# aantoine890/navierstokes

Measured on AMD Instinct MI355X. Metric: fp64 CSR SpMV GFLOP/s & % HBM roofline @ nnz; 1/2/4/8 GPU, higher is better.
Workload: dtype f64

## Files before the change

### include/mi355_devtools.h

```cpp
#ifndef MI355_DEVTOOLS_H
#define MI355_DEVTOOLS_H
#include "mi355_spmv.h"
#ifdef __cplusplus
extern "C" {
#endif
int mi_debug_xcc_map(int wgs, int* host_out);
int mi_debug_touch_pages(mi_csr_t A, int stride_bytes, const void* d_extra0, long long bytes0, const void* d_extra1, long long bytes1);
int mi_debug_mring_trace(mi_csr_t A, const double* d_x, double* d_y, int max_wgs, long long* host_out, int* wgs_out);
int mi_debug_move_array(mi_csr_t A, int which, int how, unsigned long long* old_ptr, unsigned long long* new_ptr);
int mi_debug_mring_replan(mi_csr_t A, int skew_pct, int* table_len, int* longest_run);
int mi_debug_part_push_trace(mi_part_t P, double* d_x_ext, double* d_y_local, int max_wgs, long long* host_out, int* wgs_out, int* halo_out);
int mi_debug_part_ext_mode(mi_part_t P, int mode);
int mi_debug_part_ext_trace(mi_part_t P, double* d_x_ext, double* d_y_local, int max_wgs, long long* host_out, int* wgs_out, int* modes_out);
int mi_part_push_debug_preset(mi_part_t P, unsigned value);

#ifdef __cplusplus
}
#endif
#endif
```

### navierstokes_amd/csrc/capi_bcsr.hip

```cpp
#include "capi_internal.hpp"
#include "spmv_bcsr_sell.hpp"

static int sell_fill(mi_bcsr4_t A, hipStream_t s);

template <class Select>
static bool bcsr4_race(mi_bcsr4_t A, int ncand, Select select, double* us)
{
    LaunchTimer tm;
    ScratchPair sp;
    if (sp.alloc(4 * (size_t)std::max(A->nbcols, 1), 4 * (size_t)std::max(A->nbrows, 1)) != MI_OK || tm.init() != MI_OK) return false;
    std::vector<char> failed((size_t)ncand, 0);
    for (int round = 0; round < 2; round++)
        for (int c = 0; c < ncand; c++) {
            if (failed[c]) continue;
            select(c);
            double t = 0.0;
            if (tm.time(3, 8, [&] { return launch_bcsr4(A, sp.x, sp.y, nullptr, false); }, &t) == MI_OK) us[c] = min_measured(us[c], t);
            else failed[c] = 1;
        }
    for (int c = 0; c < ncand; c++)
        if (failed[c]) us[c] = 0.0;
    return true;
}

// ... 68 lines not shown
    A->sell_nsteps = P.nsteps;
    return sell_fill(A, nullptr);
}

static void choose_bcsr4_sell_form(mi_bcsr4_t A, bool forced)
{
    if (const char* fe = getenv("MI355_BCSR_SELL_FORM")) A->sell_form = std::max(0, std::min(3, atoi(fe)));
    else if (forced) A->sell_form = 0;
    else if (env_is("MI355_SPMV_AUTOTUNE", "0")) A->sell_form = 0;
    else {
        double us[5] = {0, 0, 0, 0, 0};
        if (!bcsr4_race(A, 5, [&](int c) { A->sell_form = c - 1; }, us)) return;
        int best = 0;
        for (int c = 1; c < 5; c++) {
            A->tune_us_sell[c - 1] = us[c];
            if (better(us[c], us[best])) best = c;
        }
        if (A->tune_us_plain <= 0 && A->tune_us_tile <= 0) A->tune_us_plain = us[0];
        A->sell_form = best - 1;
    }
}

extern "C" int mi_bcsr4_create(int nbrows, int nbcols, const int* ptrow, const int* indcol, const double* coef,
                               mi_bcsr4_t* out)
{
    CHECK_ARG(out, "out is null");
    *out = nullptr;
    CHECK_ARG(nbrows >= 0 && nbcols >= 0 && ptrow && ptrow[0] == 0, "bad argument");
    for (int i = 0; i < nbrows; i++) CHECK_ARG(ptrow[i] <= ptrow[i + 1], "ptrow must be non-decreasing");
    const long long nb = ptrow[nbrows];
    CHECK_ARG(nb == 0 || (indcol && coef), "indcol/coef is null");
    for (long long k = 0; k < nb; k++) CHECK_ARG(indcol[k] >= 0 && indcol[k] < nbcols, "block column outside [0, nbcols)");
    int rc = need_device();
    if (rc) return rc;
    std::unique_ptr<mi_bcsr4_s, int (*)(mi_bcsr4_t)> owner(new (std::nothrow) mi_bcsr4_s(), mi_bcsr4_destroy);
    mi_bcsr4_t A = owner.get();
    if (!A) return fail(MI_ERR_ALLOC, "host allocation failed");
    A->nbrows = nbrows;
    A->nbcols = nbcols;
    A->nblocks = nb;
    hipError_t e;
    if ((e = hipGetDevice(&A->device)) != hipSuccess ||
        (e = hipMalloc(&A->d_ptrow, sizeof(int) * ((size_t)nbrows + 1))) != hipSuccess ||
        (e = hipMalloc(&A->d_indcol, sizeof(int) * ((size_t)nb + 1))) != hipSuccess ||
        (e = hipMalloc(&A->d_coef, sizeof(double) * 16 * ((size_t)nb + 1))) != hipSuccess ||
        (e = hipMemcpy(A->d_ptrow, ptrow, sizeof(int) * ((size_t)nbrows + 1), hipMemcpyHostToDevice)) != hipSuccess ||
        (nb && (e = hipMemcpy(A->d_indcol, indcol, sizeof(int) * (size_t)nb, hipMemcpyHostToDevice)) != hipSuccess) ||
        (nb && (e = hipMemcpy(A->d_coef, coef, sizeof(double) * 16 * (size_t)nb, hipMemcpyHostToDevice)) != hipSuccess))
        return fail(e == hipErrorOutOfMemory ? MI_ERR_ALLOC : MI_ERR_HIP, std::string("bcsr4 upload: ") + hipGetErrorString(e));
    for (int s0 = 0; s0 < nbrows; s0 += kSellRows)
        A->max_slice_vals = std::max(A->max_slice_vals, 16 * (ptrow[std::min(nbrows, s0 + kSellRows)] - ptrow[s0]));
    if ((rc = build_bcsr4_tile(A, ptrow, indcol))) return rc;
    const bool forced = env_is("MI355_BCSR_SELL", "1");
    if (!env_is("MI355_BCSR_SELL", "0") && (forced || nb >= 100000) && nbcols > 0 && nbcols < (1 << 30)) {
        if ((rc = build_bcsr4_sell(A, ptrow, indcol))) return rc;
        if (A->d_sell_val) choose_bcsr4_sell_form(A, forced);
    }
    if ((e = hipStreamSynchronize(nullptr)) != hipSuccess) return fail(MI_ERR_HIP, std::string("mi_bcsr4_create: ") + hipGetErrorString(e));
    *out = owner.release();
    return MI_OK;
}

static int sell_fill(mi_bcsr4_t A, hipStream_t s)
{
    const int grid = std::max(1, std::min(A->sell_nslices, 8192));
    hipLaunchKernelGGL(bcsr4_to_sell_kernel, dim3((unsigned)grid), dim3(64), 0, s, A->sell_nslices, A->nbrows, A->d_ptrow, A->d_coef, A->d_sell_sptr, A->d_sell_val);
    HIP_TRY(hipGetLastError());
    return MI_OK;
}

int bcsr4_refresh_from_csr(mi_bcsr4_s* A, const int* d_csr_ptrow, const double* d_src, double* d_csr_out, hipStream_t s)
{
    if (!A || A->nbrows == 0) return MI_OK;
    const int nslices = (A->nbrows + kSellRows - 1) / kSellRows;
    const int grid = std::max(1, std::min(nslices, 2048));
    const int* sptr = A->d_sell_val ? A->d_sell_sptr : nullptr;
    double* sv = A->d_sell_val;
    if (A->max_slice_vals <= 4096)
        hipLaunchKernelGGL((bcsr4_refresh_kernel<4096>), dim3((unsigned)grid), dim3(256), 0, s, nslices, A->nbrows, d_csr_ptrow, d_src, d_csr_out, A->d_ptrow, A->d_coef, sptr, sv);
    else if (A->max_slice_vals <= 16384)
        hipLaunchKernelGGL((bcsr4_refresh_kernel<16384>), dim3((unsigned)std::min(grid, 256)), dim3(256), 0, s, nslices, A->nbrows, d_csr_ptrow, d_src, d_csr_out, A->d_ptrow, A->d_coef, sptr, sv);
    else
        hipLaunchKernelGGL((bcsr4_refresh_kernel<0>), dim3((unsigned)grid), dim3(256), 0, s, nslices, A->nbrows, d_csr_ptrow, d_src, d_csr_out, A->d_ptrow, A->d_coef, sptr, sv);
    HIP_TRY(hipGetLastError());
    return MI_OK;
}

static int bcsr4_refresh_from_blocks(mi_bcsr4_s* A, const double* d_src, bool colmajor, hipStream_t s)
{
    if (!A || A->nbrows == 0 || A->nblocks == 0) return MI_OK;
    const int nslices = (A->nbrows + kSellRows - 1) / kSellRows;
    const int grid = std::max(1, std::min(nslices, 2048));
    const int* sptr = A->d_sell_val ? A->d_sell_sptr : nullptr;
    double* out = d_src == A->d_coef ? nullptr : A->d_coef;
    if (colmajor && !out) return fail(MI_ERR_ARG, "column-major blocks cannot be transposed in place");
    if (!out && !A->d_sell_val) return MI_OK;
#define BR_LAUNCH(CAP_, CM_, G_) hipLaunchKernelGGL((bcsr4_blocks_refresh_kernel<CAP_, CM_>), dim3((unsigned)(G_)), dim3(256), 0, s, nslices, A->nbrows, A->d_ptrow, d_src, out, sptr, A->d_sell_val)
    if (A->max_slice_vals <= 4096) { if (colmajor) BR_LAUNCH(4096, true, grid); else BR_LAUNCH(4096, false, grid); }
    else if (A->max_slice_vals <= 16384) { if (colmajor) BR_LAUNCH(16384, true, std::min(grid, 256)); else BR_LAUNCH(16384, false, std::min(grid, 256)); }
    else { if (colmajor) BR_LAUNCH(0, true, grid); else BR_LAUNCH(0, false, grid); }
#undef BR_LAUNCH
    HIP_TRY(hipGetLastError());
    return MI_OK;
}

int bcsr4_values_changed(mi_bcsr4_s* A, hipStream_t s)
{
    if (A && A->d_sell_val && A->nblocks > 0) return sell_fill(A, s);
    return MI_OK;
}

extern "C" int mi_bcsr4_sell_info(mi_bcsr4_t A, int* built, int* form_in_use, long long* steps, double* padding, double us[4])
{
    CHECK_ARG(A, "null handle");
    if (built) *built = A->d_sell_val != nullptr;
    if (form_in_use) *form_in_use = A->d_sell_val ? A->sell_form : -1;
    if (steps) *steps = A->sell_nsteps;
    if (padding) *padding = A->nblocks > 0 && A->d_sell_val ? (double)A->sell_nsteps * kSellRows / (double)A->nblocks - 1.0 : 0.0;
    if (us)
        for (int i = 0; i < 4; i++) us[i] = A->tune_us_sell[i];
    return MI_OK;
}

extern "C" int mi_bcsr4_sell_plan_probe(int nbrows, const int* ptrow, const int* indcol, int nwaves_max, int* nslices, long long* nsteps,
                                        int* nwaves, int* sptr, int* wrng, unsigned* col)
{
    CHECK_ARG(nbrows >= 0 && ptrow && ptrow[0] == 0 && nwaves_max >= 1, "bad argument");
    for (int i = 0; i < nbrows; i++) CHECK_ARG(ptrow[i] <= ptrow[i + 1], "ptrow must be non-decreasing");
    const long long nb = ptrow[nbrows];
    CHECK_ARG(nb == 0 || indcol, "indcol is null");
    for (long long k = 0; k < nb; k++) CHECK_ARG(indcol[k] >= 0 && indcol[k] < (1 << 30), "block column outside [0, 2^30)");
    SellPlanHost P;
    build_sell_plan(nbrows, ptrow, indcol, nwaves_max, P);
    if (nslices) *nslices = P.nslices;
    if (nsteps) *nsteps = P.nsteps;
    if (nwaves) *nwaves = P.nwaves;
    if (sptr) std::copy(P.sptr.begin(), P.sptr.end(), sptr);
    if (wrng) std::copy(P.wrng.begin(), P.wrng.end(), wrng);
    if (col) std::copy(P.col.begin(), P.col.end(), col);
    return MI_OK;
}

static void transpose_blocks_host(long long nb, const double* src, double* dst)
{
    for (long long k = 0; k < nb; k++)
        for (int r = 0; r < 4; r++)
            for (int c = 0; c < 4; c++) dst[16 * k + 4 * r + c] = src[16 * k + 4 * c + r];
}

extern "C" int mi_bcsr4_create_layout(int nbrows, int nbcols, const int* ptrow, const int* indcol, const double* coef, int layout,
                                      mi_bcsr4_t* out)
{
    CHECK_ARG(layout == MI_BLOCK_ROWMAJOR || layout == MI_BLOCK_COLMAJOR, "unknown block layout");
    if (layout == MI_BLOCK_ROWMAJOR) return mi_bcsr4_create(nbrows, nbcols, ptrow, indcol, coef, out);
    CHECK_ARG(out, "out is null");
    *out = nullptr;
    CHECK_ARG(nbrows >= 0 && ptrow && ptrow[0] == 0 && ptrow[nbrows] >= 0, "bad argument");
    const long long nb = ptrow[nbrows];
    CHECK_ARG(nb == 0 || coef, "coef is null");
    std::vector<double> t((size_t)nb * 16);
    transpose_blocks_host(nb, coef, t.data());
    return mi_bcsr4_create(nbrows, nbcols, ptrow, indcol, t.data(), out);
}

extern "C" int mi_bcsr4_update_values_layout(mi_bcsr4_t A, const double* coef, int layout)
{
// ... 605 lines not shown
```

### navierstokes_amd/csrc/capi_csr.hip

```cpp
#include "capi_internal.hpp"
#include "reorder.hpp"
#include "mring_plan.hpp"
#include "tile_plan.hpp"

int get_table(mi_csr_t A, int nnzb, BlockTable** out)
{
    BlockTable& T = A->tables[nnzb];
    if (!T.d_blk) {
        std::vector<int> rows, ptrs;
        int row_align = A->nnz < 20000000 ? 64 : 1;
        if (const char* e = getenv("MI355_STREAM_ROW_ALIGN")) row_align = std::max(1, atoi(e));
        build_row_blocks(A->n, A->h_ptrow.data(), nnzb, 4 * kWG, rows, ptrs, row_align, 7);
        T.nnzb = nnzb;
        T.nblk = (int)rows.size() - 1;
        std::vector<int2> h(rows.size());
        for (size_t i = 0; i < rows.size(); i++) h[i] = make_int2(rows[i], ptrs[i]);
        HIP_TRY(hipMalloc(&T.d_blk, sizeof(int2) * h.size()));
        HIP_TRY(hipMemcpy(T.d_blk, h.data(), sizeof(int2) * h.size(), hipMemcpyHostToDevice));
    }
    *out = &T;
    return MI_OK;
}

static void free_tile(mi_csr_t A)
{
    dfree(A->tile.d_desc);
    dfree(A->tile.d_ulist);
    dfree(A->tile.d_slots);
    A->tile = TileTable();
}

static void free_mring(mi_csr_t A)
{
    dfree(A->mring.d_plan);
    dfree(A->mring.d_first);
    dfree(A->mring.d_ok);
    dfree(A->mring.d_rng);
    dfree(A->mring.d_slots);
    A->mring = MringTable();
}

static void free_sstream(mi_csr_t A)
{
    ss_free(A->ss.dev);
    A->ss = SstreamTable();
}

static inline bool beyond_infinity_cache(double bytes_per_nnz, long long nnz, int n) { return bytes_per_nnz * (double)nnz + 16.0 * (double)n > 0.75 * 256e6; }

constexpr double kSsMaxPadding = 0.12;
static double ss_max_padding()
{
    if (const char* e = getenv("MI355_SSTREAM_MAX_PADDING")) return std::max(0.0, atof(e));
    return kSsMaxPadding;
}

static int build_sstream(mi_csr_t A, const int* ptrow, const int* indcol, int ghost_lo = 0, int ghost_hi = 0)
{
    if (A->ss.dev.val) return MI_OK;
    SsPlanHost P;
    SsMwPlanHost M;
    const int shift = (A->y_offset & 1) && !A->d_rowmap ? 1 : 0;
    build_sstream_plan(A->n, A->ncols, ptrow, indcol, ss_max_padding(), P, true, shift, ghost_lo, ghost_hi);
    SstreamTable& T = A->ss;
    hipError_t e;
    if (!P.eligible) {
        if (ghost_lo < ghost_hi || env_is("MI355_SSTREAM_MW", "0")) return MI_OK;
        build_sstream_mw_plan(A->n, A->ncols, ptrow, indcol, ss_max_padding(), M, shift);
        if (!M.eligible) return MI_OK;
        e = ss_mw_upload(M, T.dev);
        T.mw = e == hipSuccess;
    } else e = ss_upload(P, T.dev, ghost_lo < ghost_hi);
    const SsPlanHost& Q = P.eligible ? P : M;
    if (e != hipSuccess) {
        free_sstream(A);
        if (e == hipErrorOutOfMemory) { (void)hipGetLastError(); return MI_OK; }
        return fail(MI_ERR_HIP, std::string("sliced copy: ") + hipGetErrorString(e));
    }
    T.nwg = Q.nwg;
    T.rounds = Q.rounds;
    T.shift = Q.shift;
    T.steps = Q.steps;
    T.padding = (double)Q.pad_places / (double)A->nnz;
    T.max_slice_nnz = Q.max_slice_nnz;
    if (ghost_lo < ghost_hi) {
        T.h_wg_halo = P.wg_halo;
        T.h_wg = P.wg;
        T.fusable = P.fusable;
    }
    sstream_fill_values(T.rounds, A->n, T.shift, A->d_ptrow, A->d_coef, nullptr, T.dev.slice_step, T.dev.slice_len, T.dev.val, T.max_slice_nnz, nullptr, T.mw ? 1 : 0);
    if ((e = hipGetLastError()) != hipSuccess) {
        free_sstream(A);
        return fail(MI_ERR_HIP, std::string("sliced copy fill: ") + hipGetErrorString(e));
    }
    T.nt = beyond_infinity_cache(10.0, A->nnz, A->n);
    T.deep = T.nt;
    if (const char* fe = getenv("MI355_SSTREAM_FORM")) {
        const int f = atoi(fe);
        T.nt = (f & 1) == 0;
        T.deep = f >= 2;
    }
    return MI_OK;
}

int launch_sstream(mi_csr_t A, const double* d_x, double* d_y, const int* rowmap, hipStream_t s, const RingComm* comm)
{
    SstreamTable& T = A->ss;
    SsView S{T.dev.val, T.dev.slot, T.dev.wg, T.dev.win, T.nwg, A->n + T.shift, A->ncols, rowmap, T.shift};
    double* yy = rowmap ? d_y : d_y - T.shift;
    if (T.mw) {
        if (comm) return fail(MI_ERR_STATE, "the cut-ring sliced stream has no fused multi-GPU form");
        SsMwView V{S, T.dev.winK};
        if (T.deep) {
            if (T.nt) hipLaunchKernelGGL((spmv_sstream_mw<12, true>), dim3((unsigned)T.nwg), dim3(256), 0, s, V, d_x, yy);
            else hipLaunchKernelGGL((spmv_sstream_mw<12, false>), dim3((unsigned)T.nwg), dim3(256), 0, s, V, d_x, yy);
        } else {
            if (T.nt) hipLaunchKernelGGL((spmv_sstream_mw<8, true>), dim3((unsigned)T.nwg), dim3(256), 0, s, V, d_x, yy);
            else hipLaunchKernelGGL((spmv_sstream_mw<8, false>), dim3((unsigned)T.nwg), dim3(256), 0, s, V, d_x, yy);
        }
        HIP_TRY(hipGetLastError());
        return MI_OK;
    }
    if (comm) {
        const unsigned grid = (unsigned)(T.nwg + comm->push_wgs);
        if (T.deep) {
            if (T.nt) hipLaunchKernelGGL((spmv_sstream_fused<12, true>), dim3(grid), dim3(256), 0, s, S, d_x, yy, *comm);
            else hipLaunchKernelGGL((spmv_sstream_fused<12, false>), dim3(grid), dim3(256), 0, s, S, d_x, yy, *comm);
        } else {
            if (T.nt) hipLaunchKernelGGL((spmv_sstream_fused<8, true>), dim3(grid), dim3(256), 0, s, S, d_x, yy, *comm);
            else hipLaunchKernelGGL((spmv_sstream_fused<8, false>), dim3(grid), dim3(256), 0, s, S, d_x, yy, *comm);
        }
    } else if (T.deep) {
        if (T.nt) hipLaunchKernelGGL((spmv_sstream<12, true>), dim3((unsigned)T.nwg), dim3(256), 0, s, S, d_x, yy);
        else hipLaunchKernelGGL((spmv_sstream<12, false>), dim3((unsigned)T.nwg), dim3(256), 0, s, S, d_x, yy);
    } else {
        if (T.nt) hipLaunchKernelGGL((spmv_sstream<8, true>), dim3((unsigned)T.nwg), dim3(256), 0, s, S, d_x, yy);
        else hipLaunchKernelGGL((spmv_sstream<8, false>), dim3((unsigned)T.nwg), dim3(256), 0, s, S, d_x, yy);
    }
    HIP_TRY(hipGetLastError());
    return MI_OK;
}

static bool ring_wants_skew(int n, const int* ptrow)
{
    long long bad = 0;
    for (int i = 0; i < n; i++) {
        const int len = ptrow[i + 1] - ptrow[i];
        bad += len > 0 && (len % 16 == 0 || len == 8);
    }
    return 2 * bad > n;
}

constexpr long long kLargeNnz = 20000000;
static size_t placed_vector_len(int n, int ncols) { return (size_t)std::max(n, ncols) + 64; }
static int large_row_align(long long nnz) { return nnz >= kLargeNnz ? 1 : 0; }

static int build_mring(mi_csr_t A, const int* indcol, int row_align = 0)
{
    if (A->mring.d_plan || A->n == 0 || A->nnz == 0) return MI_OK;
    std::vector<int> back;
    if (!indcol) {
        if (!A->d_indcol) return fail(MI_ERR_STATE, "mring plan: the handle no longer holds its column indices");
        back.resize((size_t)A->nnz);
        HIP_TRY(hipMemcpy(back.data(), A->d_indcol, sizeof(int) * (size_t)A->nnz, hipMemcpyDeviceToHost));
        indcol = back.data();
    }
    MringPlanHost P;
    build_mring_plan(A->n, A->h_ptrow.data(), indcol, P, row_align);
    MringTable& M = A->mring;
    hipError_t e;
    if ((e = hipMalloc(&M.d_plan, sizeof(int) * P.plan.size())) != hipSuccess ||
        (e = hipMalloc(&M.d_first, sizeof(int) * P.first.size())) != hipSuccess ||
        (e = hipMemcpy(M.d_first, P.first.data(), sizeof(int) * P.first.size(), hipMemcpyHostToDevice)) != hipSuccess ||
// ... 92 lines not shown
    RING_TRY(hipMemcpy(R.d_plan, best.plan.data(), sizeof(int) * best.plan.size(), hipMemcpyHostToDevice));
    RING_TRY(hipMalloc(&R.d_ok, sizeof(int) * best.run_ok.size()));
    RING_TRY(hipMemcpy(R.d_ok, best.run_ok.data(), sizeof(int) * best.run_ok.size(), hipMemcpyHostToDevice));
    R.all_in_loop = true;
    for (int g = 0; g < best.wgs; g++) R.all_in_loop = R.all_in_loop && best.run_ok[g] == 1;
    R.h_dep_ptr.clear();
    R.h_dep_run.clear();
    if (square && row_min && R.all_in_loop && R.lean && best.cfg.id == 4 && !ghosts) build_run_deps(best, n, R.h_dep_ptr, R.h_dep_run);
    for (int g = 0; g < best.wgs; g++)
        R.uniform = R.uniform && best.run_rng[2 * g] == std::min(best.nblk, g * best.bpw) &&
                    best.run_rng[2 * g + 1] == std::min(best.nblk, (g + 1) * best.bpw);
    RING_TRY(hipMalloc(&R.d_rng, sizeof(int) * best.run_rng.size()));
    RING_TRY(hipMemcpy(R.d_rng, best.run_rng.data(), sizeof(int) * best.run_rng.size(), hipMemcpyHostToDevice));
    if (ghosts) {
        R.h_run_halo = best.run_halo;
        RING_TRY(hipMalloc(&R.d_run_halo, sizeof(int) * best.run_halo.size()));
        RING_TRY(hipMemcpy(R.d_run_halo, best.run_halo.data(), sizeof(int) * best.run_halo.size(), hipMemcpyHostToDevice));
    }
    {
        std::vector<unsigned short> slots;
        build_ring_slots(best, indcol, slots);
        RING_TRY(hipMalloc(&R.d_slots, sizeof(unsigned short) * slots.size()));
        RING_TRY(hipMemcpy(R.d_slots, slots.data(), sizeof(unsigned short) * slots.size(), hipMemcpyHostToDevice));
    }
#undef RING_TRY
    R.skew = ring_wants_skew(n, ptrow);
    if (const char* e2 = getenv("MI355_RING_SKEW")) R.skew = atoi(e2) != 0;
    return MI_OK;
}

static int time_on(LaunchTimer& tm, mi_csr_t A, const double* x, double* y, int warm, int timed, double* us)
{
    return tm.time(warm, timed, [&] { return launch_spmv(A, x, y, nullptr); }, us);
}

static int placement_draws(mi_csr_t A, double* tx, double* ty, bool keep_pair)
{
    const long long nnz = A->nnz;
    const char* pe = getenv("MI355_PLACEMENT_DRAWS");
    int draws = pe ? std::max(0, std::min(16, atoi(pe))) : 4;
    const bool early_stop = pe == nullptr;
    if (!pe) {
        size_t mem_free = 0, mem_total = 0;
        if (hipMemGetInfo(&mem_free, &mem_total) == hipSuccess && nnz > 0)
            draws = (int)std::min<size_t>((size_t)draws, mem_free / 8 / (sizeof(double) * (size_t)nnz));
        else (void)hipGetLastError();
    }
    const bool blocked_choice = A->auto_kernel == MI_KERNEL_BCSR4 && A->blocked && A->blocked->d_coef && !(A->blocked->sell_form >= 0 && A->blocked->d_sell_val);
    const bool streams_coef = A->auto_kernel == MI_KERNEL_RING || A->auto_kernel == MI_KERNEL_MRING || A->auto_kernel == MI_KERNEL_STREAM || A->auto_kernel == MI_KERNEL_TILE || blocked_choice;
    if (!(draws > 0 && streams_coef && nnz >= kLargeNnz)) return MI_OK;
    LaunchTimer tm;
    ScratchPair own;
    if (!tx || !ty) {
        const size_t len = std::max(placed_vector_len(A->n, A->ncols), (size_t)(A->n_out > 0 ? A->n_out : 1));
        if (int rc = own.alloc(len, len)) return rc;
        tx = own.x;
        ty = own.y;
    }
    if (int rc = tm.init()) return rc;
    auto time_now = [&](double* us) { return time_on(tm, A, tx, ty, 3, 8, us); };
    auto redraw = [&](void** slot, size_t bytes, size_t pad_bytes, int ndraws) {
        double best = 0.0;
        if (!*slot || bytes == 0 || time_now(&best) != MI_OK) return;
        const double first = best;
        A->place_us.push_back(best);
        std::vector<void*> losers;
        for (int d = 0; d < ndraws; d++) {
            void* fresh = nullptr;
            if (hipMalloc(&fresh, bytes + pad_bytes) != hipSuccess) { (void)hipGetLastError(); break; }
            if ((pad_bytes && hipMemset((char*)fresh + bytes, 0, pad_bytes) != hipSuccess) ||
                hipMemcpy(fresh, *slot, bytes, hipMemcpyDeviceToDevice) != hipSuccess) { (void)hipGetLastError(); dfree(fresh); break; }
            std::swap(*slot, fresh);
            double t = 0.0;
            const int rct = time_now(&t);
            A->place_us.push_back(rct == MI_OK ? t : -1.0);
            if (rct == MI_OK && t < 0.96 * best) best = t;
            else std::swap(*slot, fresh);
            losers.push_back(fresh);
            if (early_stop && d == 0 && rct == MI_OK && std::fabs(t - first) <= 0.02 * first) break;
        }
        for (void* l : losers) dfree(l);
    };
    if (blocked_choice) redraw((void**)&A->blocked->d_coef, sizeof(double) * 16 * (size_t)A->blocked->nblocks, sizeof(double) * 16, draws);
    else redraw((void**)&A->d_coef, sizeof(double) * (size_t)nnz, sizeof(double) * (size_t)kRingPadNnz, draws);
    A->place_draws_coef = (int)A->place_us.size();
    if (A->auto_kernel == MI_KERNEL_RING) redraw((void**)&A->ring.d_slots, sizeof(unsigned short) * (size_t)A->ring.nblk * A->ring.cfg.nnzb, 0, (draws + 1) / 2);
    else if (A->auto_kernel == MI_KERNEL_MRING) redraw((void**)&A->mring.d_slots, sizeof(unsigned short) * (size_t)A->mring.nblk * kMringNnzb, 0, (draws + 1) / 2);
    if (keep_pair && !A->kept_x) {
        A->kept_x = tx;
        A->kept_y = ty;
        if (tx == own.x) own.hand_over();
    }
    return MI_OK;
}

constexpr long long kMeasureNnz = 200000;

struct CsrInput {
    int n, ncols;
    const int* ptrow;
    const int* indcol;
    const double* coef;
    const int* rowmap;
    int ghost_lo, ghost_hi;
    long long nnz = 0;
    bool offset_only = false;
    std::vector<int> row_min, row_max;
    bool ghosts() const { return ghost_lo < ghost_hi; }
};

static int check_input(CsrInput& in)
{
    const int n = in.n;
    const int* ptrow = in.ptrow;
    CHECK_ARG(n >= 0 && in.ncols >= 0, "negative dimension");
    CHECK_ARG(ptrow, "ptrow is null");
    CHECK_ARG(ptrow[0] == 0, "ptrow[0] must be 0");
    for (int i = 0; i < n; i++) CHECK_ARG(ptrow[i] <= ptrow[i + 1], "ptrow must be non-decreasing");
    in.nnz = ptrow[n];
    CHECK_ARG(in.nnz == 0 || (in.indcol && in.coef), "indcol/coef is null");
    CHECK_ARG(in.nnz <= 0x7fffffffLL - 2 * kRingPadNnz && n <= 0x7fffffff - 2 * kRingPadRows, "matrix too large for 32-bit offsets: partition it (mi_part_*)");
    in.row_min.resize((size_t)n);
    in.row_max.resize((size_t)n);
    for (int i = 0; i < n; i++) {
        int lo = 0x7fffffff, hi = -1;
        for (int k = ptrow[i]; k < ptrow[i + 1]; k++) {
            const int c = in.indcol[k];
            CHECK_ARG(c >= 0 && c < in.ncols, "column index outside [0, ncols)");
            lo = c < lo ? c : lo;
            hi = c > hi ? c : hi;
        }
        in.row_min[i] = lo;
        in.row_max[i] = hi;
    }
    in.offset_only = in.rowmap != nullptr && n > 0;
    for (int i = 1; in.offset_only && i < n; i++) in.offset_only = in.rowmap[i] == in.rowmap[0] + i;
    return MI_OK;
}

static int upload(mi_csr_t A, const CsrInput& in)
{
    const int n = in.n;
    const long long nnz = in.nnz;
    const size_t pad = 8, padv = kRingPadNnz, padr = kRingPadRows;
    HIP_TRY(hipGetDevice(&A->device));
    HIP_TRY(hipMalloc(&A->d_ptrow, sizeof(int) * ((size_t)n + 1 + padr)));
    HIP_TRY(hipMalloc(&A->d_indcol, sizeof(int) * ((size_t)nnz + pad)));
    HIP_TRY(hipMalloc(&A->d_coef, sizeof(double) * ((size_t)nnz + padv)));
    HIP_TRY(hipMemset(A->d_ptrow + n + 1, 0, sizeof(int) * padr));
    HIP_TRY(hipMemset(A->d_indcol + nnz, 0, sizeof(int) * pad));
    HIP_TRY(hipMemset(A->d_coef + nnz, 0, sizeof(double) * padv));
    HIP_TRY(hipMemcpy(A->d_ptrow, in.ptrow, sizeof(int) * ((size_t)n + 1), hipMemcpyHostToDevice));
    if (nnz) {
        HIP_TRY(hipMemcpy(A->d_indcol, in.indcol, sizeof(int) * (size_t)nnz, hipMemcpyHostToDevice));
        HIP_TRY(hipMemcpy(A->d_coef, in.coef, sizeof(double) * (size_t)nnz, hipMemcpyHostToDevice));
    }
    A->mapped = in.rowmap != nullptr;
    if (in.offset_only) A->y_offset = in.rowmap[0];
    if (in.rowmap && n > 0 && !in.offset_only) {
        HIP_TRY(hipMalloc(&A->d_rowmap, sizeof(int) * ((size_t)n + padr)));
        HIP_TRY(hipMemset(A->d_rowmap + n, 0, sizeof(int) * padr));
        HIP_TRY(hipMemcpy(A->d_rowmap, in.rowmap, sizeof(int) * (size_t)n, hipMemcpyHostToDevice));
    }
    return MI_OK;
}

static int plan_ring(mi_csr_t A, const CsrInput& in)
// ... 203 lines not shown
static void compare_ring_shapes(mi_csr_t A, const CsrInput& in, LaunchTimer& tm, const ScratchPair& sp)
{
    const long long nnz = in.nnz;
    if (!env_is("MI355_RING_SHAPE_COMPARE", "1") || getenv("MI355_RING_ROW_ALIGN") || nnz < kLargeNnz) return;
    auto time_now = [&](double* us) { return time_on(tm, A, sp.x, sp.y, 3, 8, us); };
    double us64 = 0.0, us1 = 0.0;
    if (A->auto_kernel == MI_KERNEL_RING && A->ring.cfg.id == 4) {
        RingPlanHost alt;
        build_ring_plan(kRingConfigs[3], in.n, in.ptrow, in.row_min.data(), in.row_max.data(), alt, in.ghost_lo, in.ghost_hi, 64);
        RingTable T2;
        if (1.0 - (double)alt.bad_nnz / (double)nnz >= 0.90 &&
            fill_ring_table(T2, alt, in.n, in.ptrow, in.indcol, nnz, in.ghosts(), in.row_min.data(), in.row_max.data(), in.n == in.ncols) == MI_OK) {
            T2.nt = A->ring.nt;
            A->kernel = MI_KERNEL_RING;
            int rct = time_now(&us1);
            std::swap(A->ring, T2);
            if (rct == MI_OK) rct = time_now(&us64);
            A->kernel = MI_KERNEL_AUTO;
            A->tune_us_ring_aligned = us64;
            A->tune_us_ring_unaligned = us1;
            if (rct != MI_OK || !(us64 < 0.98 * us1)) std::swap(A->ring, T2);
            free_ring_table(T2);
        }
    } else if (A->auto_kernel == MI_KERNEL_MRING) {
        MringTable keep = A->mring;
        A->mring = MringTable();
        if (build_mring(A, in.indcol, 64) == MI_OK && A->mring.d_plan && A->mring.ok_fraction >= 0.90) {
            A->mring.nt = keep.nt;
            A->kernel = MI_KERNEL_MRING;
            int rct = time_now(&us64);
            std::swap(A->mring, keep);
            if (rct == MI_OK) rct = time_now(&us1);
            A->kernel = MI_KERNEL_AUTO;
            A->tune_us_ring_aligned = us64;
            A->tune_us_ring_unaligned = us1;
            if (rct == MI_OK && us64 < 0.98 * us1) std::swap(A->mring, keep);
        } else {
            std::swap(A->mring, keep);
        }
        std::swap(A->mring, keep);
        free_mring(A);
        A->mring = keep;
    }
}

static int measure_at_create(mi_csr_t A, const CsrInput& in, bool defer_placement)
{
    const size_t scratch_len = placed_vector_len(in.n, in.ncols);
    LaunchTimer tm;
    ScratchPair sp;
    int rc = sp.alloc(std::max(scratch_len, (size_t)(in.ncols > 0 ? in.ncols : 1)), std::max(scratch_len, (size_t)(A->n_out > 0 ? A->n_out : 1)));
    if (rc || (rc = tm.init())) return rc;
    tune(A, tm, sp);
    compare_ring_shapes(A, in, tm, sp);
    if (!defer_placement && placement_draws(A, sp.x, sp.y, !in.rowmap && in.n == in.ncols && in.n == A->n_out && !in.ghosts()) == MI_OK &&
        A->kept_x == sp.x)
        sp.hand_over();
    return MI_OK;
}

int csr_create_impl(int n, int ncols, const int* ptrow, const int* indcol, const double* coef,
                    const int* rowmap, mi_csr_t* out, int ghost_lo, int ghost_hi, bool defer_placement)
{
    CHECK_ARG(out, "out is null");
    *out = nullptr;
    CsrInput in{n, ncols, ptrow, indcol, coef, rowmap, ghost_lo, ghost_hi};
    int rc = check_input(in);
    if (rc || (rc = need_device())) return rc;
    std::unique_ptr<mi_csr_s, int (*)(mi_csr_t)> owner(new (std::nothrow) mi_csr_s(), mi_csr_destroy);
    mi_csr_t A = owner.get();
    if (!A) return fail(MI_ERR_ALLOC, "host allocation failed");
    A->n = n;
    A->ncols = ncols;
    A->nnz = in.nnz;
    A->ghost_lo = ghost_lo;
    A->ghost_hi = ghost_hi;
    A->h_ptrow.assign(ptrow, ptrow + n + 1);
    if ((rc = upload(A, in)) || (rc = plan_ring(A, in)) || (rc = plan_optional(A, in)) || (rc = attach_blocked(A, in))) return rc;
    load_defaults(A, in);
    const bool forced_kernel = apply_forced_kernel(A);
    if (!forced_kernel && in.nnz < kMeasureNnz && A->auto_kernel == MI_KERNEL_RING && !in.ghosts()) A->auto_kernel = MI_KERNEL_STREAM;
    if (!forced_kernel && !env_is("MI355_SPMV_AUTOTUNE", "0") && in.nnz >= kMeasureNnz && (rc = measure_at_create(A, in, defer_placement))) return rc;
    HIP_TRY(hipStreamSynchronize(nullptr));
    *out = owner.release();
    return MI_OK;
}

static int time_handle(mi_csr_t A, int warm, int timed, double* us)
{
    LaunchTimer tm;
    ScratchPair sp;
    int rc = sp.alloc((size_t)(A->ncols > 0 ? A->ncols : 1), (size_t)(A->n_out > 0 ? A->n_out : 1));
    if (rc || (rc = tm.init())) return rc;
    return time_on(tm, A, sp.x, sp.y, warm, timed, us);
}

static void release_natural_arrays(mi_csr_t A)
{
    dfree(A->d_ptrow);
    dfree(A->d_indcol);
    dfree(A->d_coef);
    A->d_ptrow = A->d_indcol = nullptr;
    A->d_coef = nullptr;
    for (auto& kv : A->tables) dfree(kv.second.d_blk);
    A->tables.clear();
    free_ring_table(A->ring);
    free_tile(A);
    free_mring(A);
    free_sstream(A);
    mi_bcsr4_destroy(A->blocked);
    A->blocked = nullptr;
}

static int maybe_reorder(mi_csr_t A, const int* ptrow, const int* indcol, const double* coef)
{
    const bool force = env_is("MI355_REORDER", "1");
    if (env_is("MI355_REORDER", "0")) return MI_OK;
    const int n = A->n;
    if (A->mapped || n != A->ncols || n < 8 || A->nnz == 0) return MI_OK;
    if (!force && (n < 100000 || resolve_kernel(A) == MI_KERNEL_RING || resolve_kernel(A) == MI_KERNEL_SSTREAM)) return MI_OK;
    const int block = csr_has_block4_pattern(n, ptrow, indcol) ? 4 : 1;
    const double nn = (double)n / block;
    const double spread = mean_column_distance(n, ptrow, indcol, block);
    A->spread_before = spread;
    if (!force && spread < 2.0 * std::pow(nn, 2.0 / 3.0)) return MI_OK;
    Reorder R;
    rcm_reorder(n, ptrow, indcol, block, R);
    A->reorder_block = block;
    A->spread_after = R.spread_after;
    if (!force && R.spread_after > 0.5 * spread) return MI_OK;
    std::vector<int> p2, c2, src_start;
    std::vector<double> v2;
    permute_csr(n, ptrow, indcol, coef, R, p2, c2, v2, src_start);
    mi_csr_t inner = nullptr;
    int rc = csr_create_impl(n, n, p2.data(), c2.data(), v2.data(), R.iperm.data(), &inner);
    if (rc) return rc;
    A->inner = inner;
    hipError_t e;
    if ((e = hipMalloc(&A->d_iperm, sizeof(int) * (size_t)n)) != hipSuccess ||
        (e = hipMalloc(&A->d_src_start, sizeof(int) * (size_t)n)) != hipSuccess ||
        (e = hipMalloc(&A->d_xp, sizeof(double) * (size_t)n)) != hipSuccess ||
        (e = hipMemcpy(A->d_iperm, R.iperm.data(), sizeof(int) * (size_t)n, hipMemcpyHostToDevice)) != hipSuccess ||
        (e = hipMemcpy(A->d_src_start, src_start.data(), sizeof(int) * (size_t)n, hipMemcpyHostToDevice)) != hipSuccess)
        return fail(e == hipErrorOutOfMemory ? MI_ERR_ALLOC : MI_ERR_HIP, std::string("reorder upload: ") + hipGetErrorString(e));
    bool keep = true;
    if (!force && !env_is("MI355_SPMV_AUTOTUNE", "0")) {
        const int timed = A->nnz < 40000000 ? 12 : 6;
        A->inner = nullptr;
        rc = time_handle(A, 3, timed, &A->us_natural);
        A->inner = inner;
        if (rc) return rc;
        if ((rc = time_handle(A, 3, timed, &A->us_reordered))) return rc;
        keep = A->us_reordered < 0.97 * A->us_natural;
    }
    if (!keep) {
        mi_csr_destroy(A->inner);
        A->inner = nullptr;
        dfree(A->d_iperm);
        dfree(A->d_src_start);
        dfree(A->d_xp);
        A->d_iperm = A->d_src_start = nullptr;
        A->d_xp = nullptr;
        return MI_OK;
    }
    A->h_iperm = R.iperm;
    A->xp_claimed = false;
    release_natural_arrays(A);
    return MI_OK;
}

extern "C" int mi_csr_create(int n, int ncols, const int* ptrow, const int* indcol, const double* coef, mi_csr_t* out)
{
    int rc = csr_create_impl(n, ncols, ptrow, indcol, coef, nullptr, out, 0, 0, true);
    if (rc) return rc;
    if ((rc = maybe_reorder(*out, ptrow, indcol, coef)) || (!(*out)->inner && (rc = placement_draws(*out, nullptr, nullptr, n == ncols))) ||
        (hipStreamSynchronize(nullptr) != hipSuccess && (rc = fail(MI_ERR_HIP, "mi_csr_create: synchronize")))) {
        mi_csr_destroy(*out);
        *out = nullptr;
    }
    return rc;
}

extern "C" int mi_reorder_probe(int n, const int* ptrow, const int* indcol, int* block, int* perm, double* spread_before,
                                double* spread_after)
{
    CHECK_ARG(n >= 0 && ptrow && (ptrow[n] == 0 || indcol), "bad argument");
    for (int i = 0; i < n; i++) {
        CHECK_ARG(ptrow[i] <= ptrow[i + 1], "ptrow must be non-decreasing");
        for (int k = ptrow[i]; k < ptrow[i + 1]; k++) CHECK_ARG(indcol[k] >= 0 && indcol[k] < n, "column index outside [0, n)");
    }
    const int b = csr_has_block4_pattern(n, ptrow, indcol) ? 4 : 1;
    Reorder R;
    rcm_reorder(n, ptrow, indcol, b, R);
    if (block) *block = b;
    if (perm)
        for (int i = 0; i < n; i++) perm[i] = R.perm[i];
    if (spread_before) *spread_before = R.spread_before;
    if (spread_after) *spread_after = R.spread_after;
    return MI_OK;
}

extern "C" int mi_csr_reorder_info(mi_csr_t A, int* reordered, int* block, double* spread_before, double* spread_after,
                                   double* us_natural, double* us_reordered)
{
    CHECK_ARG(A, "null handle");
    if (reordered) *reordered = A->inner ? 1 : 0;
    if (block) *block = A->reorder_block;
    if (spread_before) *spread_before = A->spread_before;
    if (spread_after) *spread_after = A->spread_after;
    if (us_natural) *us_natural = A->us_natural;
    if (us_reordered) *us_reordered = A->us_reordered;
    return MI_OK;
}

extern "C" int mi_csr_perm(mi_csr_t A, int* reordered, int* perm)
{
    CHECK_ARG(A, "null handle");
    if (reordered) *reordered = A->inner ? 1 : 0;
    if (perm) {
        if (A->inner) {
            CHECK_ARG((int)A->h_iperm.size() == A->n, "permutation not kept on this handle");
            for (int r = 0; r < A->n; r++) perm[A->h_iperm[r]] = r;
        } else {
            for (int i = 0; i < A->n; i++) perm[i] = i;
        }
    }
    return MI_OK;
}

extern "C" int mi_vec_to_internal_dev(mi_csr_t A, const double* d_x, double* d_x_int, mi_stream_t s)
{
    CHECK_ARG(A, "null handle");
    if (A->n == 0) return MI_OK;
    CHECK_ARG(d_x && d_x_int && d_x != d_x_int, "null vector, or in place");
    if (A->inner) return gather_perm(A, d_x, d_x_int, (hipStream_t)s);
    HIP_TRY(hipMemcpyAsync(d_x_int, d_x, sizeof(double) * (size_t)A->n, hipMemcpyDeviceToDevice, (hipStream_t)s));
    return MI_OK;
}

extern "C" int mi_vec_from_internal_dev(mi_csr_t A, const double* d_x_int, double* d_x, mi_stream_t s)
{
    CHECK_ARG(A, "null handle");
    if (A->n == 0) return MI_OK;
    CHECK_ARG(d_x && d_x_int && d_x != d_x_int, "null vector, or in place");
    if (A->inner) return scatter_perm(A, d_x_int, d_x, (hipStream_t)s);
    HIP_TRY(hipMemcpyAsync(d_x, d_x_int, sizeof(double) * (size_t)A->n, hipMemcpyDeviceToDevice, (hipStream_t)s));
    return MI_OK;
}

extern "C" int mi_spmv_internal_dev(mi_csr_t A, const double* d_x_int, double* d_y_int, mi_stream_t s)
{
    CHECK_ARG(A, "null handle");
    CHECK_ARG(A->n == A->ncols && !A->mapped, "the internal numbering is defined for square, unmapped matrices");
    CHECK_ARG(A->n == 0 || (d_x_int && d_y_int), "null vector");
    if (A->inner) return launch_spmv(A->inner, d_x_int, d_y_int, (hipStream_t)s, false);
    return launch_spmv(A, d_x_int, d_y_int, (hipStream_t)s);
}

extern "C" int mi_spmk_internal_dev(mi_csr_t A, int k, const double* d_x_int, double* const* d_y_int_out, mi_stream_t s)
{
    CHECK_ARG(A, "null handle");
    if (k < 1 || k > MI_MAX_POWERS) return fail(MI_ERR_UNSUPPORTED, "k must be in 1..MI_MAX_POWERS");
    CHECK_ARG(d_y_int_out, "null output array");
    CHECK_ARG(A->n == A->ncols && !A->mapped, "the internal numbering is defined for square, unmapped matrices");
    if (A->n == 0) return MI_OK;
    CHECK_ARG(d_x_int, "null vector");
    for (int p = 0; p < k; p++) CHECK_ARG(d_y_int_out[p], "null output vector");
    return spmk_unmapped(A->inner ? A->inner : A, k, d_x_int, d_y_int_out, (hipStream_t)s);
}

extern "C" int mi_csr_create_mapped(int n, int ncols, const int* ptrow, const int* indcol, const double* coef,
                                    const int* rowmap, mi_csr_t* out)
{
    return csr_create_impl(n, ncols, ptrow, indcol, coef, rowmap, out);
}

extern "C" int mi_csr_destroy(mi_csr_t A)
{
    if (!A) return MI_OK;
    dfree(A->d_ptrow);
    dfree(A->d_indcol);
    dfree(A->d_coef);
    dfree(A->d_rowmap);
    dfree(A->d_x);
    dfree(A->d_y);
    dfree(A->kept_x);
    dfree(A->kept_y);
    for (double* p : A->d_pow) dfree(p);
    for (auto& kv : A->tables) {
        dfree(kv.second.d_blk);
    }
    free_ring_table(A->ring);
    free_tile(A);
    free_mring(A);
    free_sstream(A);
    mi_bcsr4_destroy(A->blocked);
    mi_csr_destroy(A->inner);
    dfree(A->d_iperm);
    dfree(A->d_src_start);
    dfree(A->d_xp);
    for (auto& kv : A->xp_more) dfree(kv.second);
    dfree(A->d_vtmp);
    for (double* p : A->d_pp) dfree(p);
    spmk_release(A);
    delete A;
    return MI_OK;
}

static int refresh_blocked_values(mi_csr_t A, hipStream_t s, bool sliced_done = false)
{
    if (A->ss.dev.val && !sliced_done) {
        SstreamTable& T = A->ss;
        sstream_fill_values(T.rounds, A->n, T.shift, A->d_ptrow, A->d_coef, nullptr, T.dev.slice_step, T.dev.slice_len, T.dev.val, T.max_slice_nnz, s, T.mw ? 1 : 0);
        HIP_TRY(hipGetLastError());
    }
    if (!A->blocked || A->blocked->nbrows == 0) return MI_OK;
    return bcsr4_refresh_from_csr(A->blocked, A->d_ptrow, A->d_coef, nullptr, s);
}

__global__ __launch_bounds__(256) void permute_values_kernel(int n, const int* __restrict__ new_ptrow, const int* __restrict__ src_start,
                                                             const double* __restrict__ src, double* __restrict__ dst)
{
    __shared__ int s_p[65], s_a[64];
    const int tid = threadIdx.x;
    for (int r0 = blockIdx.x * 64; r0 < n; r0 += gridDim.x * 64) {
        const int nr = min(64, n - r0);
        if (tid <= nr) s_p[tid] = new_ptrow[r0 + tid];
        if (tid < nr) s_a[tid] = src_start[r0 + tid];
        __syncthreads();
        const int b0 = s_p[0], seg = s_p[nr] - b0;
        for (int k = tid; k < seg; k += 256) {
            const int p = b0 + k;
            int lo = 0, hi = nr;
            while (hi - lo > 1) {
                const int mid = (lo + hi) >> 1;
                if (s_p[mid] <= p) lo = mid;
                else hi = mid;
            }
            dst[p] = src[s_a[lo] + (p - s_p[lo])];
        }
        __syncthreads();
    }
}

extern "C" int mi_csr_update_values_dev(mi_csr_t A, const double* d_coef, mi_stream_t s_)
{
    CHECK_ARG(A, "null handle");
    if (A->nnz == 0) return MI_OK;
    CHECK_ARG(d_coef, "null coef");
    hipStream_t s = (hipStream_t)s_;
    if (A->inner) {
        mi_csr_t I = A->inner;
        hipLaunchKernelGGL(permute_values_kernel, dim3((unsigned)std::max(1, std::min((A->n + 63) / 64, 4096))), dim3(256), 0, s, A->n, I->d_ptrow, A->d_src_start, d_coef, I->d_coef);
        HIP_TRY(hipGetLastError());
        return refresh_blocked_values(I, s);
    }
    if (A->ss.dev.val && d_coef != A->d_coef) {
        SstreamTable& T = A->ss;
        sstream_fill_values(T.rounds, A->n, T.shift, A->d_ptrow, d_coef, A->d_coef, T.dev.slice_step, T.dev.slice_len, T.dev.val, T.max_slice_nnz, s, T.mw ? 1 : 0);
        HIP_TRY(hipGetLastError());
        return refresh_blocked_values(A, s, true);
    }
    if (A->blocked && A->blocked->nbrows > 0 && d_coef != A->d_coef)
        return bcsr4_refresh_from_csr(A->blocked, A->d_ptrow, d_coef, A->d_coef, s);
    if (d_coef != A->d_coef) HIP_TRY(hipMemcpyAsync(A->d_coef, d_coef, sizeof(double) * (size_t)A->nnz, hipMemcpyDeviceToDevice, s));
    return refresh_blocked_values(A, s);
}

extern "C" int mi_csr_update_values(mi_csr_t A, const double* coef)
{
    CHECK_ARG(A, "null handle");
    if (A->nnz == 0) return MI_OK;
    CHECK_ARG(coef, "null coef");
    if (A->inner) {
        if (!A->d_vtmp) HIP_TRY(hipMalloc(&A->d_vtmp, sizeof(double) * (size_t)A->nnz));
        HIP_TRY(hipMemcpy(A->d_vtmp, coef, sizeof(double) * (size_t)A->nnz, hipMemcpyHostToDevice));
        int rc = mi_csr_update_values_dev(A, A->d_vtmp, nullptr);
        if (rc) return rc;
        HIP_TRY(hipStreamSynchronize(nullptr));
        return MI_OK;
    }
    HIP_TRY(hipMemcpy(A->d_coef, coef, sizeof(double) * (size_t)A->nnz, hipMemcpyHostToDevice));
    int rc = refresh_blocked_values(A, nullptr);
    if (rc) return rc;
    HIP_TRY(hipStreamSynchronize(nullptr));
    return MI_OK;
}

extern "C" int mi_csr_dims(mi_csr_t A, int* n, int* ncols, long long* nnz)
{
    CHECK_ARG(A, "null handle");
    if (n) *n = A->n;
    if (ncols) *ncols = A->ncols;
    if (nnz) *nnz = A->nnz;
    return MI_OK;
}

int resolve_kernel(const mi_csr_s* A)
{
    int k = A->kernel != MI_KERNEL_AUTO ? A->kernel : A->auto_kernel;
    if (k == MI_KERNEL_RING && !A->ring.d_plan) k = MI_KERNEL_STREAM;
    if (k == MI_KERNEL_BCSR4 && !A->blocked) k = MI_KERNEL_STREAM;
    if (k == MI_KERNEL_TILE && !A->tile.d_desc) k = MI_KERNEL_STREAM;
    if (k == MI_KERNEL_MRING && !A->mring.d_plan) k = MI_KERNEL_STREAM;
    if (k == MI_KERNEL_SSTREAM && !A->ss.dev.val) k = A->ring.d_plan && A->ring.ok_fraction >= 0.90 ? MI_KERNEL_RING : MI_KERNEL_STREAM;
    return k;
}

extern "C" int mi_csr_tune_info(mi_csr_t A, double* us_ring, double* us_stream)
{
    CHECK_ARG(A, "null handle");
    if (A->inner) A = A->inner;
    if (us_ring) *us_ring = A->tune_us[MI_KERNEL_RING][A->ring.nt];
    if (us_stream) *us_stream = A->tune_us[MI_KERNEL_STREAM][A->stream_nt];
    return MI_OK;
}

extern "C" int mi_csr_tune_detail(mi_csr_t A, double us[5], int* ring_nt, int* stream_nt)
{
    CHECK_ARG(A, "null handle");
    if (A->inner) A = A->inner;
    if (us) {
        us[0] = A->tune_us[MI_KERNEL_RING][0];
        us[1] = A->tune_us[MI_KERNEL_RING][1];
        us[2] = A->tune_us[MI_KERNEL_STREAM][0];
        us[3] = A->tune_us[MI_KERNEL_STREAM][1];
        us[4] = A->tune_us[MI_KERNEL_BCSR4][0];
    }
    if (ring_nt) *ring_nt = A->ring.nt ? 1 : 0;
    if (stream_nt) *stream_nt = A->stream_nt ? 1 : 0;
    return MI_OK;
}
extern "C" int mi_ring_plan_probe(int n, const int* ptrow, const int* indcol, int config_id, int* nblk, int* runs,
                                  int* runs_not_ringable, double* nnz_fraction_ringable, int* max_slot)
{
    CHECK_ARG(n >= 0 && ptrow && config_id >= 1 && config_id <= kNumRingConfigs, "bad argument");
    const long long nnz = ptrow[n];
    CHECK_ARG(nnz == 0 || indcol, "indcol is null");
    std::vector<int> row_min((size_t)n), row_max((size_t)n);
    for (int i = 0; i < n; i++) {
        int lo = 0x7fffffff, hi = -1;
        for (int k = ptrow[i]; k < ptrow[i + 1]; k++) {
            lo = std::min(lo, indcol[k]);
            hi = std::max(hi, indcol[k]);
        }
        row_min[i] = lo;
        row_max[i] = hi;
// ... 590 lines not shown
```

### navierstokes_amd/csrc/capi_internal.hpp

```cpp
#pragma once
#include "mi355_spmv.h"

#include <hip/hip_runtime.h>

#include <cstdio>
#include <cstdlib>
#include <cmath>
#include <chrono>
#include <cstring>
#include <map>
#include <memory>
#include <mutex>
#include <new>
#include <string>
#include <vector>

#include "partition.hpp"
#include "push_exchange.hpp"
#include "ring_plan.hpp"
#include "spmv_kernels.hpp"
#include "spmv_ring.hpp"
#include "spmv_sstream_mw.hpp"

using namespace mi355;
// ... 94 lines not shown
static inline double min_measured(double a, double b) { return a > 0 ? std::min(a, b) : b; }
static inline bool better(double a, double b) { return a > 0 && (b <= 0 || a < b); }

static inline bool stream_is_capturing(hipStream_t s)
{
    hipStreamCaptureStatus st = hipStreamCaptureStatusNone;
    if (hipStreamIsCapturing(s, &st) != hipSuccess) {
        (void)hipGetLastError();
        return false;
    }
    return st != hipStreamCaptureStatusNone;
}

struct BlockTable {
    int nnzb = 0;
    int nblk = 0;
    int2* d_blk = nullptr;
};

struct RingTable {
    RingConfig cfg{};
    int nblk = 0, wgs = 0, bpw = 0, bad_runs = 0;
    double ok_fraction = 0.0;
    int* d_plan = nullptr;
    int* d_ok = nullptr;
    int* d_rng = nullptr;
    int* d_run_halo = nullptr;
    std::vector<int> h_run_halo;
    bool uniform = true;
    bool lean = false;
    bool all_in_loop = false;
    std::vector<int> h_dep_ptr, h_dep_run;
    unsigned short* d_slots = nullptr;
    bool nt = false;
    bool skew = false;
};

struct MringTable {
    int nblk = 0, wgs = 0, nruns = 0, bpw = 0, bad_runs = 0, depth = 2;
    double ok_fraction = 0.0;
    long long restarts = 0;
    int* d_plan = nullptr;
    int* d_first = nullptr;
    int* d_ok = nullptr;
    int* d_rng = nullptr;
    unsigned short* d_slots = nullptr;
    bool nt = false, skew = false;
};

struct TileTable {
    int nblk = 0;
    int* d_desc = nullptr;
    unsigned* d_ulist = nullptr;
    unsigned short* d_slots = nullptr;
    double unique_per_nnz = 0.0;
    bool nt = false;
    bool skew = false;
};

struct SstreamTable {
    bool mw = false;
    SsDevice dev;
    int nwg = 0, rounds = 0;
    int shift = 0;
    long long steps = 0;
    double padding = 0.0;
    int max_slice_nnz = 0;
    bool nt = true;
    bool deep = true;
    bool fusable = false;
    bool asked = false;
    std::vector<int> h_wg_halo;
    std::vector<SsWg> h_wg;
    double tune_us[4] = {0, 0, 0, 0};
};

struct mi_csr_s {
    int device = 0;
    int n = 0, ncols = 0;
    long long nnz = 0;
    int* d_ptrow = nullptr;
    int* d_indcol = nullptr;
    double* d_coef = nullptr;
    int* d_rowmap = nullptr;
    bool mapped = false;
    int y_offset = 0;
    int ghost_lo = 0, ghost_hi = 0;
    std::vector<int> h_ptrow;
    std::map<int, BlockTable> tables;
    RingTable ring;
    TileTable tile;
    SstreamTable ss;
    MringTable mring;
    int kernel = MI_KERNEL_AUTO;
    int auto_kernel = MI_KERNEL_STREAM;
    std::vector<double> place_us;
    int place_draws_coef = 0;
    double *kept_x = nullptr, *kept_y = nullptr;
    double tune_us[MI_KERNEL_SSTREAM + 1][2] = {};
    double tune_us_ring_aligned = 0.0, tune_us_ring_unaligned = 0.0;
    bool stream_nt = false;
    mi_bcsr4_t blocked = nullptr;
    int n_out = 0;
    mi_csr_t inner = nullptr;
    int* d_iperm = nullptr;
    std::vector<int> h_iperm;
    int* d_src_start = nullptr;
    double* d_xp = nullptr;
    hipStream_t xp_stream = nullptr;
    bool xp_claimed = false;
    std::map<hipStream_t, double*> xp_more;
    std::vector<double*> d_pp;
    double* d_vtmp = nullptr;
    double spread_before = 0.0, spread_after = 0.0, us_natural = 0.0, us_reordered = 0.0;
    int reorder_block = 0;
    double* d_x = nullptr;
    double* d_y = nullptr;
    std::vector<double*> d_pow;
    unsigned* d_kflags = nullptr;
    int* d_kdep_ptr = nullptr;
    int* d_kdep_run = nullptr;
    unsigned kstep_epoch = 0;
    unsigned* h_ktimeouts = nullptr;
    unsigned* d_ktimeouts = nullptr;
    int kstep_setup = 0;
    int kstep_choice[9] = {0, 0, 0, 0, 0, 0, 0, 0, 0};
    double kstep_us[9][2] = {};
};

struct SpmmTilePlan {
    int rows = 0, umax = 0, ntiles = 0;
    double mean_list = 0.0;
    int* d_ptr = nullptr;
    unsigned* d_nodes = nullptr;
    unsigned short* d_slots = nullptr;
    int* d_rows = nullptr;
};

struct mi_bcsr4_s {
    int device = 0;
    int nbrows = 0, nbcols = 0;
    long long nblocks = 0;
    int* d_ptrow = nullptr;
    int* d_indcol = nullptr;
    double* d_coef = nullptr;
    int* d_browmap = nullptr;
    int* d_tl_ptr = nullptr;
    unsigned* d_tl_nodes = nullptr;
    unsigned short* d_tl_slots = nullptr;
    bool use_tile = false;
    double tune_us_plain = 0.0, tune_us_tile = 0.0;
    double* d_sell_val = nullptr;
    unsigned* d_sell_col = nullptr;
    int* d_sell_sptr = nullptr;
    int* d_sell_wrng = nullptr;
    int* d_sell_wrng2 = nullptr;
    int sell_nslices = 0, sell_nwaves = 0, sell_nwaves2 = 0;
    long long sell_nsteps = 0;
    int max_slice_vals = 0;
    int sell_form = -1;
    double tune_us_sell[4] = {0, 0, 0, 0};
    SpmmTilePlan st, st64;
    int st_state = 0;
    int spmm_choice[9] = {0, 0, 0, 0, 0, 0, 0, 0, 0};
    double spmm_us[9][5] = {};
    double* d_x = nullptr;
// ... 3 lines not shown

struct mi_part_s {
    PartPlan plan;
    mi_csr_t piece[2] = {nullptr, nullptr};
    int* d_send_idx = nullptr;
    bool finalized = false;
    int kernel = MI_KERNEL_AUTO;
    void* comm = nullptr;
    hipStream_t comm_stream = nullptr;
    hipEvent_t ev_pack = nullptr, ev_comm = nullptr;
    double* d_sendbuf = nullptr;
    unsigned* d_flags = nullptr;
    unsigned* h_timeouts = nullptr;
    unsigned* d_timeouts = nullptr;
    unsigned step_no = 0;
    bool flag_handoff = false;
    std::vector<int> ag_union;
    int ag_slice = 0;
    int* d_ag_idx = nullptr;
    int* d_ag_src = nullptr;
    double* d_ag_send = nullptr;
    double* d_ag_recv = nullptr;
    bool ag_ready = false, ag_use = false;
    void* win = nullptr;
    bool win_uncached = false, win_registered = false;
    std::string win_key;
    unsigned* win_flags = nullptr;
    double* win_data = nullptr;
    std::vector<void*> ipc_opened;
    PushLink* d_links = nullptr;
    int n_links = 0;
    int2* d_push_work = nullptr;
    int* d_link_chunks = nullptr;
    unsigned* d_tickets = nullptr;
    int n_push_work = 0;
    int* d_nb = nullptr;
    int n_nb = 0;
    unsigned push_step = 0;
    bool push_ready = false;
    mi_csr_t piece_all = nullptr;
    int* d_run_link = nullptr;
    const int* d_run_halo = nullptr;
    int npush_runs = 0;
    bool fused = false;
    bool ghost_readers = true;
    bool fused_ext = false;
    double* d_stage = nullptr;
    unsigned* d_ready = nullptr;
    int ext_wgs = 0;
    int2* d_ext_units = nullptr;
    int n_ext_units = 0;
    int n_ext_plain = 0;
    bool peer_on_my_device = false;
    bool ext_split = false;
    bool ext_csr = false;
    unsigned* d_ext_order = nullptr;
    int ext_debug = 0;
};

static inline size_t win_data_offset(int nranks) { return ((size_t)nranks * kWinFlagStride * sizeof(unsigned) + 255) / 256 * 256; }

extern std::mutex g_mu;
int get_ws(hipStream_t s, double** out);

struct Scratch {
    std::vector<double*> bufs;
    ~Scratch()
    {
        for (double* p : bufs) dfree(p);
    }
    int up(const double* h, size_t n, double** d)
    {
        *d = nullptr;
        HIP_TRY(hipMalloc(d, sizeof(double) * (n ? n : 1)));
        bufs.push_back(*d);
        if (h && n) HIP_TRY(hipMemcpy(*d, h, sizeof(double) * n, hipMemcpyHostToDevice));
        return MI_OK;
    }
};

int csr_create_impl(int n, int ncols, const int* ptrow, const int* indcol, const double* coef, const int* rowmap, mi_csr_t* out,
                    int ghost_lo = 0, int ghost_hi = 0, bool defer_placement = false);
int resolve_kernel(const mi_csr_s* A);
int get_table(mi_csr_t A, int nnzb, BlockTable** out);
int launch_spmv(mi_csr_t A, const double* d_x, double* d_y, hipStream_t s, bool use_map = true, const RingComm* comm = nullptr,
                const RingDot* dot = nullptr);
bool ring_dot_eligible(const mi_csr_s* A);
int reorder_scratch(mi_csr_t A, hipStream_t s, double** buf);
void launch_ring_cfg(const mi_csr_s* A, const CsrView& V, const double* d_x, double* d_y, hipStream_t s, const RingComm* comm, const RingDot* dot);
int spmk_unmapped(mi_csr_t H, int k, const double* d_x, double* const* d_y, hipStream_t s);
void spmk_release(mi_csr_t H);
int gather_perm(mi_csr_t A, const double* d_x, double* d_xp, hipStream_t s);
int ortho_update_from_parts(int n, int nparts, const double* parts, double alpha, const double* d_b, const double* d_x1, double* d_x3, double* d_beta_out,
                            hipStream_t s);
int scatter_perm(mi_csr_t A, const double* d_src, double* d_dst, hipStream_t s);
constexpr size_t kLdsBytesPerCU = 160 * 1024;
static inline size_t spmm_tile_lds(const SpmmTilePlan* T, int s) { return T ? (size_t)T->umax * (4 * s + 2) * sizeof(double) : (size_t)-1; }
hipError_t spmm_tile_launch(const mi_bcsr4_s* A, const SpmmTilePlan* Pl, const Bcsr4View& V, int s, int arith, const double* X, long long ldx,
                            double* Y, long long ldy, hipStream_t st);
hipError_t spmm_otile_launch(const mi_bcsr4_s* A, const SpmmTilePlan* Pl, const Bcsr4View& V, int s, int arith, bool nt, const double* X, long long ldx,
                             double* Y, long long ldy, hipStream_t st);
int part_push_window(mi_part_s* P);
void part_push_layout(const mi_part_s* P, long long* layout );
int part_push_connect_bases(mi_part_s* P, void* const* bases , const long long* layouts);
int part_ext_launch(mi_part_s* P, const double* d_x_ext, double* d_y_local, unsigned step, unsigned spin_max, hipStream_t s, unsigned long long* trace, int* grid_out);
int launch_sstream(mi_csr_t A, const double* d_x, double* d_y, const int* rowmap, hipStream_t s, const RingComm* comm = nullptr);
static inline bool sstream_y_ok(const mi_csr_s* A, const double* yy, const int* map) { return map || A->ss.mw || (((uintptr_t)(yy - A->ss.shift)) & 15) == 0; }
int bcsr4_values_changed(mi_bcsr4_s* A, hipStream_t s);
void bcsr4_drop_sliced(mi_bcsr4_s* A);
int bcsr4_refresh_from_csr(mi_bcsr4_s* A, const int* d_csr_ptrow, const double* d_src, double* d_csr_out, hipStream_t s);
int launch_bcsr4(mi_bcsr4_t A, const double* d_x, double* d_y, mi_stream_t s, bool use_map);
```

### navierstokes_amd/csrc/capi_part.hip

```cpp
#include "capi_internal.hpp"
#include "handoff_kernels.hpp"
#include "push_kernels.hpp"
#include "spmv_bcsr4_ext.hpp"
#include "rccl_loader.hpp"

static std::map<std::string, void*> g_win_registry;
static void part_comm_release(mi_part_s* P);
static int part_need_timeouts(mi_part_s* P);

static Rccl& g_rccl = rccl_state();
static_assert(MI_COMM_ID_BYTES == kCommIdBytes, "id size");

#define NCCL_TRY(expr)                                                                                  \
    do {                                                                                                \
        int r_ = (expr);                                                                                \
        if (r_ != 0) return fail(MI_ERR_HIP, std::string(#expr) + ": " + g_rccl.GetErrorString(r_));    \
    } while (0)

static void part_comm_release(mi_part_s* P)
{
    if (P->comm && g_rccl.ok) g_rccl.CommDestroy(P->comm);
    P->comm = nullptr;
    if (P->comm_stream) (void)hipStreamDestroy(P->comm_stream);
    if (P->ev_pack) (void)hipEventDestroy(P->ev_pack);
// ... 759 lines not shown
    return MI_OK;
}

extern "C" int mi_part_push_unfuse(mi_part_t P)
{
    CHECK_ARG(P, "null handle");
    if (!P->fused) return MI_OK;
    HIP_TRY(hipDeviceSynchronize());
    P->fused = P->fused_ext = false;
    dfree(P->d_run_link);
    dfree(P->d_stage);
    dfree(P->d_ready);
    dfree(P->d_ext_units);
    dfree(P->d_ext_order);
    P->d_stage = nullptr;
    P->d_ready = nullptr;
    P->d_ext_units = nullptr;
    P->d_ext_order = nullptr;
    P->ext_csr = false;
    P->d_run_link = nullptr;
    mi_csr_destroy(P->piece_all);
    P->piece_all = nullptr;
    return MI_OK;
}

extern "C" const char* mi_part_kernel_name(mi_part_t P, int which)
{
    if (!P || which < 0 || which > 2) return "";
    if (which < 2) return P->piece[which] ? mi_csr_kernel_name(P->piece[which]) : "";
    if (!P->fused || !P->piece_all) return "";
    if (P->fused_ext && P->ext_csr) return P->ext_split ? "spmv_csr_fused_ext x2 (ranks share a device: two launches)" : "spmv_csr_fused_ext";
    if (P->fused_ext) return P->ext_split ? "spmv_bcsr4_fused_ext x2 (ranks share a device: two launches)" : "spmv_bcsr4_fused_ext";
    static thread_local char nm[160];
    const char* base = mi_csr_kernel_name(P->piece_all);
    if (resolve_kernel(P->piece_all) == MI_KERNEL_SSTREAM) snprintf(nm, sizeof nm, "spmv_sstream_fused<%d, %s>", P->piece_all->ss.deep ? 12 : 8, P->piece_all->ss.nt ? "true" : "false");
    else snprintf(nm, sizeof nm, "%s [FUSED]", base);
    return nm;
}

extern "C" int mi_part_push_info(mi_part_t P, int* ready, int* fused, int* neighbours)
{
    CHECK_ARG(P, "null handle");
    if (ready) *ready = P->push_ready ? 1 : 0;
    if (fused) *fused = P->fused ? 1 : 0;
    if (neighbours) *neighbours = P->n_nb;
    return MI_OK;
}
int part_ext_launch(mi_part_s* P, const double* d_x_ext, double* d_y_local, unsigned step, unsigned spin_max, hipStream_t s, unsigned long long* trace, int* grid_out)
{
    const PartPlan& pl = P->plan;
    if (!P->ext_csr && (((uintptr_t)d_x_ext) & 15) != 0) return fail(MI_ERR_ARG, "the fused blocked step needs a 16-byte aligned x");
    ExtComm C;
    C.links = P->d_links;
    C.work = P->d_push_work;
    C.link_chunks = P->d_link_chunks;
    C.tickets = P->d_tickets;
    C.send_idx = P->d_send_idx;
    C.flags = P->win_flags;
    C.nb = P->d_nb;
    C.halo = P->win_data + (size_t)(step & 1u) * (size_t)pl.n_halo;
    C.stage = P->d_stage;
    C.ready = P->d_ready;
    C.timeouts = P->d_timeouts;
    C.n_work = P->n_push_work;
    C.n_nb = P->n_nb;
    C.n_local = pl.n_local;
    C.n_halo = pl.n_halo;
    C.xwgs = P->n_push_work + P->ext_wgs;
    C.step = step;
    C.spin_max = spin_max;
    C.trace = trace;
    C.nowait = 0;
    if (P->ext_debug & 2) C.links = nullptr;
    if (P->ext_debug & 4) C.n_halo = 0;
    if (P->ext_debug & 8) C.n_nb = 0;
    const bool split = P->ext_split && !trace && P->n_ext_units > P->n_ext_plain;
    const dim3 grid((split ? P->n_ext_plain : P->n_ext_units) + C.xwgs);
    if (grid_out) *grid_out = (int)grid.x;
    if (P->ext_csr) {
        mi_csr_t A = P->piece_all;
        BlockTable* T = nullptr;
        int rc = get_table(A, 1024, &T);
        if (rc) return rc;
        CsrView V{A->n, A->ncols, A->d_ptrow, A->d_indcol, A->d_coef, nullptr, T->d_blk, nullptr, T->nblk};
        if (trace) hipLaunchKernelGGL((spmv_csr_fused_ext<1024, false, true>), grid, dim3(kWG), 0, s, V, d_x_ext, d_y_local, C, P->d_ext_order);
        else if (A->stream_nt) hipLaunchKernelGGL((spmv_csr_fused_ext<1024, true>), grid, dim3(kWG), 0, s, V, d_x_ext, d_y_local, C, P->d_ext_order);
        else hipLaunchKernelGGL((spmv_csr_fused_ext<1024, false>), grid, dim3(kWG), 0, s, V, d_x_ext, d_y_local, C, P->d_ext_order);
        if (split) {
            ExtComm C2 = C;
            C2.xwgs = C2.n_work = 0;
            C2.nowait = 1;
            const dim3 g2(P->n_ext_units - P->n_ext_plain);
            if (A->stream_nt) hipLaunchKernelGGL((spmv_csr_fused_ext<1024, true>), g2, dim3(kWG), 0, s, V, d_x_ext, d_y_local, C2, P->d_ext_order + P->n_ext_plain);
            else hipLaunchKernelGGL((spmv_csr_fused_ext<1024, false>), g2, dim3(kWG), 0, s, V, d_x_ext, d_y_local, C2, P->d_ext_order + P->n_ext_plain);
        }
        HIP_TRY(hipGetLastError());
        return MI_OK;
    }
    mi_bcsr4_t B = P->piece_all->blocked;
    Bcsr4View V{B->nbrows, B->nbcols, B->d_ptrow, B->d_indcol, B->d_coef, nullptr};
    if (trace) {
        hipLaunchKernelGGL((spmv_bcsr4_fused_ext<kBcsrDepth, 4, kWG, true>), grid, dim3(kWG), 0, s, V, d_x_ext, d_y_local, C, P->d_ext_units);
        HIP_TRY(hipGetLastError());
        return MI_OK;
    }
    static const int depth = getenv("MI355_PUSH_EXT_DEPTH") ? atoi(getenv("MI355_PUSH_EXT_DEPTH")) : 24;
#define EXT_LAUNCH(P_, U_) hipLaunchKernelGGL((spmv_bcsr4_fused_ext<P_, U_, kWG>), grid, dim3(kWG), 0, s, V, d_x_ext, d_y_local, C, P->d_ext_units)
    switch (depth) {
    case 22: EXT_LAUNCH(2, 2); break;
    case 23: EXT_LAUNCH(2, 3); break;
    case 27: EXT_LAUNCH(2, 7); break;
    default: EXT_LAUNCH(2, 4); break;
    }
#undef EXT_LAUNCH
    if (split) {
        ExtComm C2 = C;
        C2.xwgs = C2.n_work = 0;
        C2.nowait = 1;
        hipLaunchKernelGGL((spmv_bcsr4_fused_ext<kBcsrDepth, 4, kWG>), dim3(P->n_ext_units - P->n_ext_plain), dim3(kWG), 0, s, V, d_x_ext, d_y_local, C2,
                           P->d_ext_units + P->n_ext_plain);
    }
    HIP_TRY(hipGetLastError());
    return MI_OK;
}

extern "C" int mi_part_spmv_push_dev(mi_part_t P, double* d_x_ext, double* d_y_local, mi_stream_t s_)
{
    CHECK_ARG(P, "null handle");
    if (!P->finalized) return fail(MI_ERR_STATE, "partition not finalized");
    hipStream_t s = (hipStream_t)s_;
    const PartPlan& pl = P->plan;
    int rc;
    if (pl.nranks == 1) {
        if ((rc = mi_spmv_dev(P->piece[0], d_x_ext, d_y_local, s))) return rc;
        return mi_spmv_dev(P->piece[1], d_x_ext, d_y_local, s);
    }
    if (!P->push_ready) return fail(MI_ERR_STATE, "mi_part_push_connect was not called");
    if ((rc = part_handoff_status(P))) return rc;
    if (stream_is_capturing(s))
        return fail(MI_ERR_UNSUPPORTED, "the push step cannot be captured into a HIP graph: its step number is a kernel argument (a replay would "
                                        "present an old step and every wait would pass at once); capture mi_part_spmv_dev (RCCL, events) instead");
    const unsigned step = ++P->push_step;
    static const unsigned spin_max = 1u << (getenv("MI355_PUSH_SPIN_LOG2") ? std::max(8, std::min(30, atoi(getenv("MI355_PUSH_SPIN_LOG2")))) : kPushSpinLog2Default);
    if (P->fused_ext) return part_ext_launch(P, d_x_ext, d_y_local, step, spin_max, s, nullptr, nullptr);
    if (P->fused) {
        RingComm C;
        C.links = P->d_links;
        C.send_idx = P->d_send_idx;
        C.flags = P->win_flags;
        C.nb = P->d_nb;
        C.halo = P->win_data + (size_t)(step & 1u) * (size_t)(pl.n_halo > 0 ? pl.n_halo : 1);
        C.run_halo = P->d_run_halo;
        C.timeouts = P->d_timeouts;
        C.n_links = P->n_links;
        C.n_nb = P->n_nb;
        C.n_local = pl.n_local;
        C.n_left = pl.n_left;
        C.run_link = P->d_run_link;
        C.npush_runs = P->npush_runs;
        C.push_wgs = (P->npush_runs == 0 && P->n_links > 0) ? kNXCD : 0;
        C.step = step;
        C.spin_max = spin_max;
        C.gate_push = P->ghost_readers ? 0 : 1;
        if ((rc = launch_spmv(P->piece_all, d_x_ext, d_y_local, s, true, &C))) return rc;
        return MI_OK;
    }
    if (P->n_links)
// ... 71 lines not shown
```

### navierstokes_amd/csrc/devtools.hip

```cpp
#include "capi_internal.hpp"
#include "mi355_devtools.h"

__global__ __launch_bounds__(256) void xcc_probe_kernel(int* out)
{
    __shared__ double hog[9000];
    hog[threadIdx.x] = 0.0;
    if (threadIdx.x == 0) out[blockIdx.x] = __builtin_amdgcn_s_getreg((3 << 11) | 20) & 15;
    if (hog[threadIdx.x] != 0.0) out[blockIdx.x] = -1;
}

extern "C" int mi_debug_xcc_map(int wgs, int* host_out)
{
    CHECK_ARG(wgs > 0 && host_out, "bad argument");
    int rc = need_device();
    if (rc) return rc;
    int* d = nullptr;
    HIP_TRY(hipMalloc(&d, sizeof(int) * wgs));
    hipLaunchKernelGGL(xcc_probe_kernel, dim3(wgs), dim3(256), 0, nullptr, d);
    HIP_TRY(hipMemcpy(host_out, d, sizeof(int) * wgs, hipMemcpyDeviceToHost));
    dfree(d);
    return MI_OK;
}
__global__ __launch_bounds__(256) void touch_pages_kernel(const char* __restrict__ p, size_t bytes, size_t stride, int* __restrict__ sink)
{
    int acc = 0;
    const size_t step = (size_t)gridDim.x * blockDim.x;
    for (size_t i = (size_t)blockIdx.x * blockDim.x + threadIdx.x; i * stride < bytes; i += step)
        acc += *reinterpret_cast<const int*>(p + i * stride);
    if (acc == 0x7fffffff) sink[0] = acc;
}

extern "C" int mi_debug_touch_pages(mi_csr_t A, int stride_bytes, const void* d_extra0, long long bytes0, const void* d_extra1, long long bytes1)
{
    CHECK_ARG(A && stride_bytes >= 64 && stride_bytes % 4 == 0, "bad argument");
    if (A->inner) A = A->inner;
    int* sink = nullptr;
    HIP_TRY(hipMalloc(&sink, 64));
    auto touch = [&](const void* p, size_t bytes) {
        if (!p || bytes < 4) return;
        hipLaunchKernelGGL(touch_pages_kernel, dim3(256), dim3(256), 0, nullptr, (const char*)p, bytes - 3, (size_t)stride_bytes, sink);
    };
    const size_t nnz = (size_t)A->nnz, n = (size_t)A->n;
    touch(A->d_coef, 8 * nnz);
    touch(A->d_indcol, 4 * nnz);
    touch(A->d_ptrow, 4 * (n + 1));
    touch(A->d_rowmap, 4 * n);
    if (A->ring.d_plan) {
        touch(A->ring.d_plan, 32 * (size_t)A->ring.nblk);
        touch(A->ring.d_slots, 2 * (size_t)A->ring.nblk * A->ring.cfg.nnzb);
    }
    if (A->tile.d_desc) {
        touch(A->tile.d_desc, 16 * (size_t)A->tile.nblk);
        touch(A->tile.d_ulist, (size_t)(A->tile.unique_per_nnz * 4.0 * (double)nnz));
        touch(A->tile.d_slots, 2 * nnz);
    }
    if (A->blocked) {
        touch(A->blocked->d_coef, 128 * (size_t)A->blocked->nblocks);
        touch(A->blocked->d_indcol, 4 * (size_t)A->blocked->nblocks);
        touch(A->blocked->d_ptrow, 4 * ((size_t)A->blocked->nbrows + 1));
    }
    touch(d_extra0, (size_t)bytes0);
    touch(d_extra1, (size_t)bytes1);
    HIP_TRY(hipGetLastError());
    HIP_TRY(hipDeviceSynchronize());
    dfree(sink);
    return MI_OK;
}
extern "C" int mi_part_push_debug_preset(mi_part_t P, unsigned value)
{
    CHECK_ARG(P && P->win, "no window");
    std::vector<unsigned> f((size_t)P->plan.nranks * kWinFlagStride, value);
    HIP_TRY(hipMemcpy(P->win_flags, f.data(), sizeof(unsigned) * f.size(), hipMemcpyHostToDevice));
    return MI_OK;
}

#include "spmv_mring.hpp"
extern "C" int mi_debug_mring_trace(mi_csr_t A, const double* d_x, double* d_y, int max_wgs, long long* host_out, int* wgs_out)
{
    CHECK_ARG(A && d_x && d_y && host_out && wgs_out, "null argument");
    if (A->inner) A = A->inner;
    const MringTable& M = A->mring;
    if (!M.d_plan) return fail(MI_ERR_STATE, "no multi-window ring plan on this handle");
    CHECK_ARG(M.wgs <= max_wgs, "output array too small");
    CsrView V{};
    V.n = A->n;
    V.ncols = A->ncols;
    V.ptrow = A->d_ptrow;
    V.indcol = A->d_indcol;
    V.coef = A->d_coef;
    V.rowmap = nullptr;
    V.nblk = M.nblk;
    long long* d = nullptr;
    HIP_TRY(hipMalloc(&d, sizeof(long long) * 4 * (size_t)M.wgs));
    HIP_TRY(hipMemset(d, 0, sizeof(long long) * 4 * (size_t)M.wgs));
    hipLaunchKernelGGL((spmv_csr_mring<kMringThreads, kMringNnzb, 4, kMringMaxB, false, true, false, true>), dim3(M.wgs), dim3(kMringThreads), 0, nullptr,
                       V, reinterpret_cast<const int4*>(M.d_plan), reinterpret_cast<const int4*>(M.d_first), M.d_ok, M.d_slots, d_x, d_y,
                       reinterpret_cast<const int2*>(M.d_rng), M.wgs, d);
    HIP_TRY(hipDeviceSynchronize());
    HIP_TRY(hipMemcpy(host_out, d, sizeof(long long) * 4 * (size_t)M.wgs, hipMemcpyDeviceToHost));
    dfree(d);
    *wgs_out = M.wgs;
    return MI_OK;
}

extern "C" int mi_debug_move_array(mi_csr_t A, int which, int how, unsigned long long* old_ptr, unsigned long long* new_ptr)
{
    CHECK_ARG(A && which >= 0 && which <= 3 && (how == 0 || how == 2 || how == 3), "bad argument (how = 1, hipDeviceMallocContiguous, is refused: see the comment in devtools.hip)");
    if (A->inner) A = A->inner;
    void** slot = nullptr;
    size_t bytes = 0, pad_bytes = 0;
    if (which == 0) { slot = (void**)&A->d_coef; bytes = sizeof(double) * (size_t)A->nnz; pad_bytes = sizeof(double) * (size_t)kRingPadNnz; }
    if (which == 1) { slot = (void**)&A->ring.d_slots; bytes = sizeof(unsigned short) * (size_t)A->ring.nblk * A->ring.cfg.nnzb; }
    if (which == 2) { slot = (void**)&A->d_ptrow; bytes = sizeof(int) * ((size_t)A->n + 1); pad_bytes = sizeof(int) * (size_t)kRingPadRows; }
    if (which == 3) { slot = (void**)&A->ring.d_plan; bytes = sizeof(int) * 8 * (size_t)A->ring.nblk; }
    if (!*slot || bytes == 0) return fail(MI_ERR_STATE, "the handle has no such array");
    void* fresh = nullptr;
    if (how == 0) HIP_TRY(hipMalloc(&fresh, bytes + pad_bytes));
    else HIP_TRY(hipExtMallocWithFlags(&fresh, bytes + pad_bytes, how == 2 ? hipDeviceMallocUncached : hipDeviceMallocFinegrained));
    if (pad_bytes) HIP_TRY(hipMemset((char*)fresh + bytes, 0, pad_bytes));
    HIP_TRY(hipMemcpy(fresh, *slot, bytes, hipMemcpyDeviceToDevice));
    HIP_TRY(hipDeviceSynchronize());
    if (old_ptr) *old_ptr = (unsigned long long)(uintptr_t)*slot;
    if (new_ptr) *new_ptr = (unsigned long long)(uintptr_t)fresh;
    void* old = *slot;
    *slot = fresh;
    HIP_TRY(hipFree(old));
    return MI_OK;
}

#include "mring_plan.hpp"
extern "C" int mi_debug_mring_replan(mi_csr_t A, int skew_pct, int* table_len, int* longest_run)
{
    CHECK_ARG(A, "null handle");
    if (A->inner) A = A->inner;
    MringTable& M = A->mring;
    if (!M.d_plan || !A->d_indcol) return fail(MI_ERR_STATE, "no multi-window ring plan (or no column indices) on this handle");
    std::vector<int> ind((size_t)A->nnz);
    HIP_TRY(hipMemcpy(ind.data(), A->d_indcol, sizeof(int) * (size_t)A->nnz, hipMemcpyDeviceToHost));
    MringPlanHost P;
    build_mring_plan(A->n, A->h_ptrow.data(), ind.data(), P, 0, skew_pct);
    if (P.nblk != M.nblk) return fail(MI_ERR_STATE, "the new plan has other row blocks");
    if (const char* bad = check_mring_plan(P, A->n, A->h_ptrow.data(), ind.data())) return fail(MI_ERR_STATE, std::string("mring plan: ") + bad);
    HIP_TRY(hipDeviceSynchronize());
    HIP_TRY(hipMemcpy(M.d_plan, P.plan.data(), sizeof(int) * P.plan.size(), hipMemcpyHostToDevice));
    HIP_TRY(hipMemcpy(M.d_slots, P.slots.data(), sizeof(unsigned short) * P.slots.size(), hipMemcpyHostToDevice));
    dfree(M.d_first); dfree(M.d_ok); dfree(M.d_rng);
    M.d_first = M.d_ok = M.d_rng = nullptr;
    HIP_TRY(hipMalloc(&M.d_first, sizeof(int) * P.first.size()));
    HIP_TRY(hipMalloc(&M.d_ok, sizeof(int) * P.run_ok.size()));
    HIP_TRY(hipMalloc(&M.d_rng, sizeof(int) * P.run_rng.size()));
    HIP_TRY(hipMemcpy(M.d_first, P.first.data(), sizeof(int) * P.first.size(), hipMemcpyHostToDevice));
    HIP_TRY(hipMemcpy(M.d_ok, P.run_ok.data(), sizeof(int) * P.run_ok.size(), hipMemcpyHostToDevice));
    HIP_TRY(hipMemcpy(M.d_rng, P.run_rng.data(), sizeof(int) * P.run_rng.size(), hipMemcpyHostToDevice));
    M.wgs = P.wgs;
    M.nruns = P.nruns;
    M.bpw = P.bpw;
    M.bad_runs = P.bad_runs;
    if (table_len) *table_len = P.wgs;
    if (longest_run) {
        *longest_run = 0;
        for (int g = 0; g < P.wgs; g++) *longest_run = std::max(*longest_run, P.run_rng[2 * g + 1] - P.run_rng[2 * g]);
    }
    return MI_OK;
}

extern "C" int mi_debug_part_push_trace(mi_part_t P, double* d_x_ext, double* d_y_local, int max_wgs, long long* host_out, int* wgs_out, int* halo_out)
{
    CHECK_ARG(P && d_x_ext && d_y_local && host_out && wgs_out, "null argument");
    if (!P->push_ready || !P->fused || !P->piece_all || resolve_kernel(P->piece_all) != MI_KERNEL_SSTREAM || !P->piece_all->ss.fusable)
        return fail(MI_ERR_STATE, "the one-launch push step of this handle does not run the sliced stream");
    mi_csr_t A = P->piece_all;
    SstreamTable& T = A->ss;
    CHECK_ARG(T.nwg <= max_wgs, "host buffer too small");
    const PartPlan& pl = P->plan;
    const unsigned step = ++P->push_step;
    RingComm C{};
    C.links = P->d_links;
    C.send_idx = P->d_send_idx;
    C.flags = P->win_flags;
    C.nb = P->d_nb;
    C.halo = P->win_data + (size_t)(step & 1u) * (size_t)(pl.n_halo > 0 ? pl.n_halo : 1);
    C.run_halo = P->d_run_halo;
    C.timeouts = P->d_timeouts;
    C.n_links = P->n_links;
    C.n_nb = P->n_nb;
    C.n_local = pl.n_local;
    C.n_left = pl.n_left;
    C.run_link = P->d_run_link;
    C.npush_runs = P->npush_runs;
    C.push_wgs = (P->npush_runs == 0 && P->n_links > 0) ? kNXCD : 0;
    C.step = step;
    C.spin_max = 1u << kPushSpinLog2Default;
    C.gate_push = P->ghost_readers ? 0 : 1;
    unsigned long long* d_tr = nullptr;
// ... 65 lines not shown
```

### navierstokes_amd/csrc/launch_csr.hip

```cpp
#include "capi_internal.hpp"
#include "spmv_rowpar.hpp"
#include "spmv_tile.hpp"
#include "spmv_mring.hpp"

int reorder_scratch(mi_csr_t A, hipStream_t s, double** buf)
{
    std::lock_guard<std::mutex> lock(g_mu);
    if (!A->xp_claimed || A->xp_stream == s) {
        A->xp_claimed = true;
        A->xp_stream = s;
        *buf = A->d_xp;
        return MI_OK;
    }
    double*& b = A->xp_more[s];
    if (!b) {
        if (stream_is_capturing(s)) return fail(MI_ERR_STATE, "first product of a relabelled handle on this stream: run one outside stream capture first (it allocates a gather buffer)");
        HIP_TRY(hipMalloc(&b, sizeof(double) * (size_t)A->n));
    }
    *buf = b;
    return MI_OK;
}

bool ring_dot_eligible(const mi_csr_s* A)
{
    if (A->inner || A->n == 0 || A->d_rowmap || A->y_offset) return false;
    if (resolve_kernel(A) != MI_KERNEL_RING) return false;
    const RingTable& R = A->ring;
    int depth = R.cfg.depth;
    if (const char* e = getenv("MI355_RING_DEPTH")) depth = atoi(e);
    return R.cfg.id == 4 && R.lean && depth != 3 && R.all_in_loop && R.wgs >= 1 && R.wgs <= 1024  &&
           !env_is("MI355_SPMV_DOT_EPILOGUE", "0");
}

int launch_spmv(mi_csr_t A, const double* d_x, double* d_y, hipStream_t s, bool use_map, const RingComm* comm, const RingDot* dot)
{
    if (dot && !ring_dot_eligible(A)) return fail(MI_ERR_STATE, "dot epilogue requested on a handle whose launch cannot carry it");
    if (A->n == 0) return MI_OK;
    const bool ss_fused = comm && resolve_kernel(A) == MI_KERNEL_SSTREAM && A->ss.fusable;
    if (comm && (A->inner || A->d_rowmap || (resolve_kernel(A) != MI_KERNEL_RING && !ss_fused)))
        return fail(MI_ERR_STATE, "fused multi-GPU step: the combined piece must be an unmapped, unreordered handle served by the ring or the sliced-stream kernel");
    if (A->inner) {
        double* xp = nullptr;
        int rc = reorder_scratch(A, s, &xp);
        if (rc) return rc;
        if ((rc = gather_perm(A, d_x, xp, s))) return rc;
        return launch_spmv(A->inner, xp, d_y, s, true);
    }
    int kid = resolve_kernel(A);
    if (kid == MI_KERNEL_SSTREAM && !dot && (!comm || ss_fused)) {
        const int* map = use_map ? A->d_rowmap : nullptr;
        double* yy = d_y + (use_map ? A->y_offset : 0);
        if (sstream_y_ok(A, yy, map)) return launch_sstream(A, d_x, yy, map, s, comm);
        if (comm) return fail(MI_ERR_ARG, "fused multi-GPU step: y must be 16-byte aligned");
        kid = A->ring.d_plan && A->ring.ok_fraction >= 0.90 ? MI_KERNEL_RING : MI_KERNEL_STREAM;
    } else if (kid == MI_KERNEL_SSTREAM) {
        kid = A->ring.d_plan && A->ring.ok_fraction >= 0.90 ? MI_KERNEL_RING : MI_KERNEL_STREAM;
    }
    if (use_map) d_y += A->y_offset;
    CsrView V{};
    V.n = A->n;
    V.ncols = A->ncols;
    V.ptrow = A->d_ptrow;
    V.indcol = A->d_indcol;
    V.coef = A->d_coef;
    V.rowmap = use_map ? A->d_rowmap : nullptr;
    V.blk = nullptr;
    V.blk_span = nullptr;
    V.nblk = 0;
    if (kid == MI_KERNEL_BCSR4 && (((uintptr_t)d_x) & 15) == 0) return launch_bcsr4(A->blocked, d_x, d_y, (mi_stream_t)s, use_map);
    if (kid == MI_KERNEL_BCSR4) {
        BlockTable* T = nullptr;
        int rc = get_table(A, 1024, &T);
        if (rc) return rc;
        V.blk = T->d_blk;
        V.nblk = T->nblk;
        const int grid = kNXCD * ((T->nblk + kNXCD - 1) / kNXCD);
        hipLaunchKernelGGL((spmv_csr_stream<1024, false>), dim3(grid), dim3(kWG), 0, s, V, d_x, d_y);
        HIP_TRY(hipGetLastError());
        return MI_OK;
    }
    if (kid == MI_KERNEL_MRING) {
        const MringTable& M = A->mring;
        V.nblk = M.nblk;
        const int4* plan = reinterpret_cast<const int4*>(M.d_plan);
        const int2* rng = reinterpret_cast<const int2*>(M.d_rng);
#define MRING_L(D_, MP_, NT_, SK_) hipLaunchKernelGGL((spmv_csr_mring<kMringThreads, kMringNnzb, D_, kMringMaxB, MP_, NT_, SK_>), dim3(M.wgs), dim3(kMringThreads), 0, s, V, plan, reinterpret_cast<const int4*>(M.d_first), M.d_ok, M.d_slots, d_x, d_y, rng, M.wgs)
#define MRING_L3(D_, MP_) do { if (M.nt) { if (M.skew) MRING_L(D_, MP_, true, true); else MRING_L(D_, MP_, true, false); } \
                               else { if (M.skew) MRING_L(D_, MP_, false, true); else MRING_L(D_, MP_, false, false); } } while (0)
#define MRING_L2(D_) do { if (V.rowmap) MRING_L3(D_, true); else MRING_L3(D_, false); } while (0)
        int depth = M.depth;
        if (const char* e = getenv("MI355_RING_DEPTH")) depth = atoi(e);
        if (depth == 4) MRING_L2(4);
        else MRING_L2(2);
#undef MRING_L2
#undef MRING_L3
#undef MRING_L
    } else if (kid == MI_KERNEL_TILE) {
        const TileTable& T = A->tile;
        const int grid = kNXCD * ((T.nblk + kNXCD - 1) / kNXCD);
        const int4* desc = reinterpret_cast<const int4*>(T.d_desc);
#define TILE_LAUNCH(NT_, SK_) hipLaunchKernelGGL((spmv_csr_tile<kTileNnzb, NT_, SK_>), dim3(grid), dim3(kTileThreads), 0, s, V, desc, T.nblk, T.d_ulist, T.d_slots, d_x, d_y)
        if (T.nt) { if (T.skew) TILE_LAUNCH(true, true); else TILE_LAUNCH(true, false); }
        else { if (T.skew) TILE_LAUNCH(false, true); else TILE_LAUNCH(false, false); }
#undef TILE_LAUNCH
    } else if (kid == MI_KERNEL_ROWPAR) {
        hipLaunchKernelGGL(spmv_csr_rowpar, dim3((A->n + kWG - 1) / kWG), dim3(kWG), 0, s, V, d_x, d_y);
    } else if (kid == MI_KERNEL_RING) {
        V.nblk = A->ring.nblk;
        launch_ring_cfg(A, V, d_x, d_y, s, comm, dot);
    } else {
        BlockTable* T = nullptr;
        int rc = get_table(A, 1024, &T);
        if (rc) return rc;
        V.blk = T->d_blk;
        V.nblk = T->nblk;
        const int grid = kNXCD * ((T->nblk + kNXCD - 1) / kNXCD);
        if (A->stream_nt) hipLaunchKernelGGL((spmv_csr_stream<1024, true>), dim3(grid), dim3(kWG), 0, s, V, d_x, d_y);
        else hipLaunchKernelGGL((spmv_csr_stream<1024, false>), dim3(grid), dim3(kWG), 0, s, V, d_x, d_y);
    }
    HIP_TRY(hipGetLastError());
    return MI_OK;
}
```

### navierstokes_amd/csrc/launch_spmk.hip

```cpp
#include "capi_internal.hpp"
#include "spmk_ring.hpp"

template <int D, bool NT, bool SKEW>
static hipError_t launch_fused_t(const mi_csr_s* H, const CsrView& V, const SpmkArgs& K, hipStream_t s, bool query, int* max_blocks)
{
    auto kern = spmk_csr_ring<256, 2048, 5120, D, kRingMaxB, NT, SKEW>;
    if (query) return hipOccupancyMaxActiveBlocksPerMultiprocessor(max_blocks, kern, 256, 0);
    hipLaunchKernelGGL(kern, dim3(H->ring.wgs), dim3(256), 0, s, V, reinterpret_cast<const int4*>(H->ring.d_plan), H->ring.d_slots,
                       reinterpret_cast<const int2*>(H->ring.d_rng), H->ring.uniform ? H->ring.bpw : 0, K);
    return hipGetLastError();
}

static hipError_t launch_fused(const mi_csr_s* H, const CsrView& V, const SpmkArgs& K, hipStream_t s, bool query = false, int* max_blocks = nullptr)
{
    const bool nt = H->ring.nt, sk = H->ring.skew;
    if (H->ring.cfg.depth == 4) {
        if (nt) return sk ? launch_fused_t<4, true, true>(H, V, K, s, query, max_blocks) : launch_fused_t<4, true, false>(H, V, K, s, query, max_blocks);
        return sk ? launch_fused_t<4, false, true>(H, V, K, s, query, max_blocks) : launch_fused_t<4, false, false>(H, V, K, s, query, max_blocks);
    }
    if (nt) return sk ? launch_fused_t<2, true, true>(H, V, K, s, query, max_blocks) : launch_fused_t<2, true, false>(H, V, K, s, query, max_blocks);
    return sk ? launch_fused_t<2, false, true>(H, V, K, s, query, max_blocks) : launch_fused_t<2, false, false>(H, V, K, s, query, max_blocks);
}

void spmk_release(mi_csr_t H)
{
    dfree(H->d_kflags);
    dfree(H->d_kdep_ptr);
    dfree(H->d_kdep_run);
    if (H->h_ktimeouts) (void)hipHostFree(H->h_ktimeouts);
    H->d_kflags = nullptr;
    H->d_kdep_ptr = H->d_kdep_run = nullptr;
    H->h_ktimeouts = H->d_ktimeouts = nullptr;
    H->kstep_setup = 0;
}

static CsrView unmapped_view(const mi_csr_s* H)
{
    CsrView V{};
    V.n = H->n;
    V.ncols = H->ncols;
    V.ptrow = H->d_ptrow;
    V.indcol = H->d_indcol;
    V.coef = H->d_coef;
    V.rowmap = nullptr;
    V.blk = nullptr;
    V.blk_span = nullptr;
    V.nblk = H->ring.nblk;
    return V;
}

static int spmk_setup(mi_csr_t H)
{
    if (H->kstep_setup) return H->kstep_setup;
    H->kstep_setup = -1;
    const RingTable& R = H->ring;
    const int kid = resolve_kernel(H);
    if (H->inner || H->n != H->ncols || (kid != MI_KERNEL_RING && kid != MI_KERNEL_SSTREAM) || !R.d_plan || R.ok_fraction < 0.90 || R.cfg.id != 4 || !R.lean || !R.all_in_loop ||
        R.cfg.depth == 3 || R.h_dep_ptr.empty() || R.wgs < kNXCD || R.wgs % kNXCD)
        return -1;
    int maxdep = 0;
    for (int g = 0; g < R.wgs; g++) maxdep = std::max(maxdep, R.h_dep_ptr[g + 1] - R.h_dep_ptr[g]);
    if (maxdep > 64) return -1;
    int per_cu = 0, dev = 0, cus = 0;
    SpmkArgs dummy{};
    if (launch_fused(H, unmapped_view(H), dummy, nullptr, true, &per_cu) != hipSuccess || hipGetDevice(&dev) != hipSuccess ||
        hipDeviceGetAttribute(&cus, hipDeviceAttributeMultiprocessorCount, dev) != hipSuccess) {
        (void)hipGetLastError();
        return -1;
    }
    if ((long long)per_cu * cus < R.wgs) return -1;
    hipError_t e;
    const size_t nflag = (size_t)R.wgs * kSpmkFlagStride;
    if ((e = hipMalloc(&H->d_kflags, sizeof(unsigned) * nflag)) != hipSuccess || (e = hipMemset(H->d_kflags, 0, sizeof(unsigned) * nflag)) != hipSuccess ||
        (e = hipStreamSynchronize(nullptr)) != hipSuccess ||
        (e = hipMalloc(&H->d_kdep_ptr, sizeof(int) * R.h_dep_ptr.size())) != hipSuccess ||
        (e = hipMalloc(&H->d_kdep_run, sizeof(int) * std::max<size_t>(1, R.h_dep_run.size()))) != hipSuccess ||
        (e = hipMemcpy(H->d_kdep_ptr, R.h_dep_ptr.data(), sizeof(int) * R.h_dep_ptr.size(), hipMemcpyHostToDevice)) != hipSuccess ||
        (R.h_dep_run.size() && (e = hipMemcpy(H->d_kdep_run, R.h_dep_run.data(), sizeof(int) * R.h_dep_run.size(), hipMemcpyHostToDevice)) != hipSuccess) ||
        (e = hipHostMalloc((void**)&H->h_ktimeouts, sizeof(unsigned), hipHostMallocMapped)) != hipSuccess) {
        (void)hipGetLastError();
        spmk_release(H);
        H->kstep_setup = -1;
        return -1;
    }
    *H->h_ktimeouts = 0;
    if (hipHostGetDevicePointer((void**)&H->d_ktimeouts, H->h_ktimeouts, 0) != hipSuccess) {
        spmk_release(H);
        H->kstep_setup = -1;
        return -1;
    }
    H->kstep_epoch = 0;
    H->kstep_setup = 1;
    return 1;
}

static int spmk_chain(mi_csr_t H, int k, const double* d_x, double* const* d_y, hipStream_t s)
{
    const double* src = d_x;
    for (int p = 0; p < k; p++) {
        int rc = launch_spmv(H, src, d_y[p], s, false);
        if (rc) return rc;
        src = d_y[p];
    }
    return MI_OK;
}

static int spmk_fused(mi_csr_t H, int k, const double* d_x, double* const* d_y, hipStream_t s)
{
    SpmkArgs K{};
    K.x = d_x;
    for (int p = 0; p < k; p++) K.y[p] = d_y[p];
    for (int p = k; p < kSpmkFusedMaxK; p++) K.y[p] = d_y[k - 1];
    K.k = k;
    K.epoch = H->kstep_epoch;
    H->kstep_epoch += (unsigned)k;
    K.flags = H->d_kflags;
    K.dep_ptr = H->d_kdep_ptr;
    K.dep_run = H->d_kdep_run;
    K.timeouts = H->d_ktimeouts;
    static const unsigned spin_max = 1u << (getenv("MI355_SPMK_SPIN_LOG2") ? std::max(8, std::min(30, atoi(getenv("MI355_SPMK_SPIN_LOG2")))) : 21);
    K.spin_max = spin_max;
    K.acquire = env_is("MI355_SPMK_ACQUIRE", "1") ? 1 : 0;
    hipError_t e = launch_fused(H, unmapped_view(H), K, s);
    if (e != hipSuccess) return fail(MI_ERR_HIP, std::string("one-launch powers step: ") + hipGetErrorString(e));
    return MI_OK;
}

int spmk_unmapped(mi_csr_t H, int k, const double* d_x, double* const* d_y, hipStream_t s)
{
    if (H->h_ktimeouts && __atomic_load_n(H->h_ktimeouts, __ATOMIC_ACQUIRE) != 0)
        return fail(MI_ERR_HIP, "mi_spmk: a hand-off wait of the one-launch powers step gave up (workgroups of the grid were not all resident); "
                                "results since then are invalid — set MI355_SPMK_FUSED=0 when other kernels share the GPU");
    if (k < 2 || k > kSpmkFusedMaxK || env_is("MI355_SPMK_FUSED", "0") || stream_is_capturing(s) || spmk_setup(H) != 1) return spmk_chain(H, k, d_x, d_y, s);
    if (env_is("MI355_SPMK_FUSED", "1")) return spmk_fused(H, k, d_x, d_y, s);
    if (H->kstep_choice[k] == 0) {
        LaunchTimer tm(s);
        if (tm.init() != MI_OK) {
            (void)hipGetLastError();
            return spmk_chain(H, k, d_x, d_y, s);
        }
        double us[2] = {0, 0};
        int rc = MI_OK;
        for (int round = 0; round < 2 && !rc; round++)
            for (int form = 0; form < 2 && !rc; form++) {
                double t = 0.0;
                rc = tm.time(2, 5, [&] { return form ? spmk_fused(H, k, d_x, d_y, s) : spmk_chain(H, k, d_x, d_y, s); }, &t);
                if (!rc) us[form] = min_measured(us[form], t);
                if (form == 1 && H->h_ktimeouts && __atomic_load_n(H->h_ktimeouts, __ATOMIC_ACQUIRE) != 0) round = 2;
            }
        if (rc) return rc;
        H->kstep_us[k][0] = us[0];
        H->kstep_us[k][1] = us[1];
        const bool gave_up = H->h_ktimeouts && __atomic_load_n(H->h_ktimeouts, __ATOMIC_ACQUIRE) != 0;
        if (gave_up) *H->h_ktimeouts = 0;
        H->kstep_choice[k] = (!gave_up && us[1] > 0 && us[1] < 0.98 * us[0]) ? 1 : -1;
    }
    return H->kstep_choice[k] == 1 ? spmk_fused(H, k, d_x, d_y, s) : spmk_chain(H, k, d_x, d_y, s);
}

extern "C" int mi_csr_spmk_info(mi_csr_t A, int k, int* eligible, int* one_launch, double* us_k_launches, double* us_one_launch)
{
    CHECK_ARG(A && k >= 1 && k <= MI_MAX_POWERS, "bad argument");
    mi_csr_t H = A->inner ? A->inner : A;
    const bool small = k <= kSpmkFusedMaxK;
    if (eligible) *eligible = small && k >= 2 && H->kstep_setup == 1;
    if (one_launch) *one_launch = small && (env_is("MI355_SPMK_FUSED", "1") ? H->kstep_setup == 1 : H->kstep_choice[k] == 1);
    if (us_k_launches) *us_k_launches = small ? H->kstep_us[k][0] : 0.0;
    if (us_one_launch) *us_one_launch = small ? H->kstep_us[k][1] : 0.0;
    return MI_OK;
}
```

### navierstokes_amd/csrc/spmv_bcsr_sell.hpp

```cpp
#pragma once
#include <hip/hip_runtime.h>

#include <algorithm>
#include <vector>

#include "spmv_kernels.hpp"

namespace mi355 {

constexpr int kSellRows = 16;
constexpr int kSellStepDoubles = 256;
constexpr int kSellPadSteps = 48;
constexpr unsigned kSellPadCol = 0x80000000u;
constexpr unsigned kSellFirstCol = 0x40000000u;
constexpr unsigned kSellColMask = 0x3fffffffu;

struct SellView {
    const double* val;
    const unsigned* col;
    const int* sptr;
    const int* wrng;
    int nslices, nbrows;
    const int* browmap = nullptr;
};
// ... 44 lines not shown
    for (int w = 1; w < W; w++) {
        const long long target = steps * w / W;
        while (s < NS && P.sptr[s] < target) s++;
        wrng[w] = s;
    }
}

typedef double sell_v2d __attribute__((ext_vector_type(2)));

template <bool NT>
__device__ __forceinline__ sell_v2d sell_ld(const sell_v2d* p)
{
    return NT ? __builtin_nontemporal_load(p) : *p;
}

__global__ __launch_bounds__(64) void bcsr4_to_sell_kernel(int nslices, int nbrows, const int* __restrict__ ptrow, const double* __restrict__ coef,
                                                           const int* __restrict__ sptr, double* __restrict__ val)
{
    const int lane = threadIdx.x, r = lane >> 2, q = lane & 3;
    for (int s = blockIdx.x; s < nslices; s += gridDim.x) {
        const int bi = kSellRows * s + r;
        const int b0 = bi < nbrows ? ptrow[bi] : 0, n = bi < nbrows ? ptrow[bi + 1] - b0 : 0;
        const int t0 = sptr[s], L = sptr[s + 1] - t0;
        for (int j = 0; j < L; j++) {
            sell_v2d lo = {0.0, 0.0}, hi = {0.0, 0.0};
            if (j < n) {
                const sell_v2d* src = reinterpret_cast<const sell_v2d*>(coef + 16 * (size_t)(b0 + j) + 4 * q);
                lo = src[0];
                hi = src[1];
            }
            sell_v2d* dst = reinterpret_cast<sell_v2d*>(val + (size_t)(t0 + j) * kSellStepDoubles);
            dst[lane] = lo;
            dst[64 + lane] = hi;
        }
    }
}

template <int CAP>
__global__ __launch_bounds__(256) void bcsr4_refresh_kernel(int nslices, int nbrows, const int* __restrict__ csr_ptrow, const double* __restrict__ src,
                                                            double* __restrict__ csr_out, const int* __restrict__ bptr, double* __restrict__ bval,
                                                            const int* __restrict__ sptr, double* __restrict__ sell_val)
{
    __shared__ double buf[CAP > 0 ? CAP : 1];
    __shared__ int rp[4 * kSellRows + 1];
    __shared__ int bp[kSellRows + 1];
    const int tid = threadIdx.x;
    for (int s = blockIdx.x; s < nslices; s += gridDim.x) {
        if (tid <= 4 * kSellRows) rp[tid] = csr_ptrow[min(4 * kSellRows * s + tid, 4 * nbrows)];
        if (tid <= kSellRows) bp[tid] = bptr[min(kSellRows * s + tid, nbrows)];
        __syncthreads();
        const int base = rp[0], seg = rp[4 * kSellRows] - base;
        const bool staged = CAP > 0 && seg <= CAP;
        if (staged) {
            for (int k0 = tid; k0 < seg; k0 += 4 * 256) {
                double v[4];
#pragma unroll
                for (int u = 0; u < 4; u++) v[u] = src[base + min(k0 + 256 * u, seg - 1)];
#pragma unroll
                for (int u = 0; u < 4; u++)
                    if (k0 + 256 * u < seg) {
                        buf[k0 + 256 * u] = v[u];
                        if (csr_out) csr_out[base + k0 + 256 * u] = v[u];
                    }
            }
            __syncthreads();
        } else if (csr_out) {
            for (int k = tid; k < seg; k += 256) csr_out[base + k] = src[base + k];
        }
        auto at = [&](int row, int pos) -> double { return staged ? buf[rp[row] - base + pos] : src[rp[row] + pos]; };
        for (int r = 0; r < kSellRows; r++) {
            const int nb = bp[r + 1] - bp[r];
            for (int k = tid; k < 16 * nb; k += 256) bval[16 * (size_t)bp[r] + k] = at(4 * r + ((k >> 2) & 3), 4 * (k >> 4) + (k & 3));
        }
        if (sell_val) {
            const int t0 = sptr[s], L = sptr[s + 1] - t0;
            for (int k = tid; k < L * 128; k += 256) {
                const int j = k >> 7, h = (k >> 6) & 1, lane = k & 63, r = lane >> 2, q = lane & 3;
                sell_v2d v = {0.0, 0.0};
                if (j < bp[r + 1] - bp[r]) {
                    v.x = at(4 * r + q, 4 * j + 2 * h);
                    v.y = at(4 * r + q, 4 * j + 2 * h + 1);
                }
                reinterpret_cast<sell_v2d*>(sell_val + (size_t)(t0 + j) * kSellStepDoubles)[h * 64 + lane] = v;
            }
        }
        __syncthreads();
    }
}

template <int CAP, bool COLMAJOR>
__global__ __launch_bounds__(256) void bcsr4_blocks_refresh_kernel(int nslices, int nbrows, const int* __restrict__ bptr, const double* __restrict__ src,
                                                                   double* __restrict__ bval_out, const int* __restrict__ sptr, double* __restrict__ sell_val)
{
    __shared__ double buf[CAP > 0 ? CAP : 1];
    __shared__ int bp[kSellRows + 1];
    const int tid = threadIdx.x;
    for (int s = blockIdx.x; s < nslices; s += gridDim.x) {
        if (tid <= kSellRows) bp[tid] = bptr[min(kSellRows * s + tid, nbrows)];
        __syncthreads();
        const size_t base = 16 * (size_t)bp[0];
        const int seg = 16 * (bp[kSellRows] - bp[0]);
        const bool staged = CAP > 0 && seg <= CAP;
        const bool copy_in_stage = staged && !COLMAJOR && bval_out != nullptr;
        if (staged) {
            for (int k0 = tid; k0 < seg; k0 += 4 * 256) {
                double v[4];
#pragma unroll
                for (int u = 0; u < 4; u++) v[u] = src[base + min(k0 + 256 * u, seg - 1)];
#pragma unroll
                for (int u = 0; u < 4; u++)
                    if (k0 + 256 * u < seg) {
                        buf[k0 + 256 * u] = v[u];
                        if (copy_in_stage) bval_out[base + k0 + 256 * u] = v[u];
                    }
            }
            __syncthreads();
        }
        auto el = [&](int blk, int q, int c) -> double {
            const int o = 16 * blk + (COLMAJOR ? 4 * c + q : 4 * q + c);
            return staged ? buf[o] : src[base + o];
        };
        if (bval_out && !copy_in_stage)
            for (int k = tid; k < seg; k += 256) bval_out[base + k] = el(k >> 4, (k >> 2) & 3, k & 3);
        if (sell_val) {
            const int t0 = sptr[s], L = sptr[s + 1] - t0;
            for (int k = tid; k < L * 128; k += 256) {
                const int j = k >> 7, h = (k >> 6) & 1, lane = k & 63, r = lane >> 2, q = lane & 3;
                sell_v2d v = {0.0, 0.0};
                if (j < bp[r + 1] - bp[r]) {
                    const int blk = bp[r] - bp[0] + j;
                    v.x = el(blk, q, 2 * h);
                    v.y = el(blk, q, 2 * h + 1);
                }
                reinterpret_cast<sell_v2d*>(sell_val + (size_t)(t0 + j) * kSellStepDoubles)[h * 64 + lane] = v;
            }
        }
        __syncthreads();
    }
}

constexpr int kSellPark = 32;
template <int D, bool NT, int ABL = 0, int YM = 0, int NW = 4>
__global__ __launch_bounds__(64 * NW) void spmv_bcsr4_sell(SellView S, const double* __restrict__ x, double* __restrict__ y, int nwg)
{
    __shared__ double s_park[YM == 2 ? NW * kSellPark * 64 : 1];
    __shared__ int s_pid[YM == 2 ? NW * kSellPark : 1];
    double* park = s_park + (YM == 2 ? ((int)threadIdx.x >> 6) * kSellPark * 64 + ((int)threadIdx.x & 63) : 0);
    int* pid = s_pid + (YM == 2 ? ((int)threadIdx.x >> 6) * kSellPark : 0);
    int parked = 0;
    const int per = nwg >> 3;
    const int lwg = per > 0 && (nwg & 7) == 0 ? ((int)blockIdx.x & 7) * per + ((int)blockIdx.x >> 3) : (int)blockIdx.x;
    const int wave = __builtin_amdgcn_readfirstlane(lwg * NW + ((int)threadIdx.x >> 6));
    const int lane = threadIdx.x & 63, r = lane >> 2;
    const sell_v2d* vbase = reinterpret_cast<const sell_v2d*>(S.val) + lane;
    const unsigned* cbase = S.col + r;

    auto flush = [&]() {
        for (int j = 0; j < parked; j++) {
            const int bj = kSellRows * pid[j] + r;
            if (bj < S.nbrows) y[4 * (size_t)(S.browmap ? S.browmap[bj] : bj) + (lane & 3)] = park[j * 64];
        }
        parked = 0;
    };
    auto emit = [&](int sl, double v) {
        const int bi = kSellRows * sl + r;
        double* dst = y + 4 * (size_t)((S.browmap && bi < S.nbrows) ? S.browmap[bi] : bi) + (lane & 3);
// ... 210 lines not shown
```

### navierstokes_amd/csrc/spmv_sstream.hpp

```cpp
#pragma once
#include <hip/hip_runtime.h>

#include <algorithm>
#include <thread>
#include <vector>

#include "spmv_ring.hpp"

namespace mi355 {

typedef double ss_v2d __attribute__((ext_vector_type(2)));
constexpr int kSsRing = 8192;
constexpr int kSsSliceRows = 128;
constexpr int kSsRound = 512;
constexpr int kSsNewMax = 1024;
constexpr int kSsPark = 20;
#ifndef MI355_SS_TAIL
#define MI355_SS_TAIL 2
#endif
constexpr int kSsTail = MI355_SS_TAIL;
constexpr unsigned kSsPad = 0x8000u;
constexpr unsigned kSsFirst = 0x4000u;
constexpr int kSsPadSteps = 64;
constexpr int kSsMaxWgs = 256;
// ... 247 lines not shown
                for (int v = row0; v < std::min(nv, row0 + kSsSliceRows); v++) L = std::max(L, PT(v + 1) - PT(v));
                if (L != P.slice_len[(size_t)r * 4 + wv]) return "slice length disagrees with the rows";
                for (int j = 0; j < L; j++)
                    for (int l = 0; l < 64; l++) {
                        const unsigned s = P.slot[base + (size_t)j * 64 + l];
                        if (l == 0 && ((s & kSsFirst) != 0) != (j == 0)) return "slice-begin flag misplaced";
                        for (int h = 0; h < 2; h++) {
                            const int v = row0 + 2 * l + h;
                            const unsigned sh = (s >> (16 * h)) & 0xffffu;
                            const bool real = v < nv && j < PT(v + 1) - PT(v);
                            if (!real) {
                                if (!(sh & kSsPad)) return "a padding place is not flagged";
                                continue;
                            }
                            const int c = indcol[PT(v) + j];
                            if (sh & kSsPad) return "a nonzero is flagged as padding";
                            if ((sh & (kSsRing - 1)) != (unsigned)(c & (kSsRing - 1))) return "slot is not the column's ring slot";
                            if (c < wlo || c >= whi) return "a column lies outside the window when its round runs";
                            names_ghost = names_ghost || (ghost_lo < ghost_hi && (c < ghost_lo || c >= ghost_hi));
                        }
                    }
            }
        }
        if (names_ghost && !P.wg_halo[g]) return "a workgroup names a ghost column and is not marked";
        if (P.fusable && P.wg_halo[g])
            for (int r = P.rptr[g] + 1; r < P.rptr[g + 1]; r++)
                if (P.win[r].y != 0) return "a ghost-reading workgroup takes columns in after its first fill";
        if (W.halo != P.wg_halo[g]) return "a workgroup record's ghost mark disagrees with the plan's";
    }
    return nullptr;
}

template <int CAP>
__global__ __launch_bounds__(256) void sstream_fill_kernel(int nslices, int n, int shift, const int* __restrict__ ptrow, const double* __restrict__ src,
                                                           double* __restrict__ csr_out, const int* __restrict__ slice_step, const int* __restrict__ slice_len,
                                                           ss_v2d* __restrict__ val, int pair64)
{
    __shared__ double buf[CAP > 0 ? CAP : 1];
    __shared__ int rp[kSsSliceRows + 1];
    const int tid = threadIdx.x;
    for (int sidx = blockIdx.x; sidx < nslices; sidx += gridDim.x) {
        const int row0 = kSsSliceRows * sidx - shift;
        if (tid <= kSsSliceRows) rp[tid] = ptrow[max(0, min(row0 + tid, n))];
        __syncthreads();
        const int base = rp[0], seg = rp[kSsSliceRows] - base;
        const bool staged = CAP > 0 && seg <= CAP;
        if (staged) {
            for (int k = tid; k < seg; k += 256) {
                const double v = src[base + k];
                buf[k] = v;
                if (csr_out) csr_out[base + k] = v;
            }
            __syncthreads();
        } else if (csr_out) {
            for (int k = tid; k < seg; k += 256) csr_out[base + k] = src[base + k];
        }
        const int t0 = slice_step[sidx], L = slice_len[sidx];
        for (int q = tid; q < L * 64; q += 256) {
            const int j = q >> 6, lane = q & 63;
            const int ra = pair64 ? lane : 2 * lane, rb = pair64 ? lane + 64 : 2 * lane + 1;
            const int a0 = rp[ra], a1 = rp[ra + 1], b0 = rp[rb], b1 = rp[rb + 1];
            ss_v2d v = {0.0, 0.0};
            if (j < a1 - a0) v.x = staged ? buf[a0 - base + j] : src[a0 + j];
            if (j < b1 - b0) v.y = staged ? buf[b0 - base + j] : src[b0 + j];
            val[(size_t)(t0 + j) * 64 + lane] = v;
        }
        __syncthreads();
    }
}

inline void sstream_fill_values(int rounds, int n, int shift, const int* d_ptrow, const double* d_src, double* d_csr_out, const int* d_slice_step,
                                const int* d_slice_len, ss_v2d* d_val, int max_slice_nnz, hipStream_t s, int pair64 = 0)
{
    const int nslices = 4 * rounds;
    if (nslices <= 0) return;
    if (max_slice_nnz <= 2048)
        hipLaunchKernelGGL((sstream_fill_kernel<2048>), dim3((unsigned)std::min(nslices, 2048)), dim3(256), 0, s, nslices, n, shift, d_ptrow, d_src, d_csr_out, d_slice_step, d_slice_len, d_val, pair64);
    else if (max_slice_nnz <= 8192)
        hipLaunchKernelGGL((sstream_fill_kernel<8192>), dim3((unsigned)std::min(nslices, 1024)), dim3(256), 0, s, nslices, n, shift, d_ptrow, d_src, d_csr_out, d_slice_step, d_slice_len, d_val, pair64);
    else
        hipLaunchKernelGGL((sstream_fill_kernel<0>), dim3((unsigned)std::min(nslices, 2048)), dim3(256), 0, s, nslices, n, shift, d_ptrow, d_src, d_csr_out, d_slice_step, d_slice_len, d_val, pair64);
}

struct SsDevice {
    ss_v2d* val = nullptr;
    unsigned* slot = nullptr;
    SsWg* wg = nullptr;
    int2* win = nullptr;
    int* slice_step = nullptr;
    int* slice_len = nullptr;
    int* wg_halo = nullptr;
    int2* winK = nullptr;
};
inline void ss_free(SsDevice& Dv)
{
    (void)hipFree(Dv.winK);
    (void)hipFree(Dv.val); (void)hipFree(Dv.slot); (void)hipFree(Dv.wg); (void)hipFree(Dv.win); (void)hipFree(Dv.slice_step); (void)hipFree(Dv.slice_len); (void)hipFree(Dv.wg_halo);
    Dv = SsDevice();
}
inline hipError_t ss_upload(const SsPlanHost& P, SsDevice& Dv, bool ghosts)
{
    hipError_t e;
    const size_t vbytes = sizeof(ss_v2d) * (size_t)(P.steps + kSsPadSteps) * 64;
    if ((e = hipMalloc(&Dv.val, vbytes)) != hipSuccess || (e = hipMalloc(&Dv.slot, sizeof(unsigned) * P.slot.size())) != hipSuccess ||
        (e = hipMalloc(&Dv.wg, sizeof(SsWg) * P.wg.size())) != hipSuccess || (e = hipMalloc(&Dv.win, sizeof(int2) * P.win.size())) != hipSuccess ||
        (e = hipMalloc(&Dv.slice_step, sizeof(int) * P.slice_step.size())) != hipSuccess || (e = hipMalloc(&Dv.slice_len, sizeof(int) * P.slice_len.size())) != hipSuccess ||
        (ghosts && (e = hipMalloc(&Dv.wg_halo, sizeof(int) * P.wg_halo.size())) != hipSuccess) ||
        (e = hipMemset((char*)Dv.val + sizeof(ss_v2d) * (size_t)P.steps * 64, 0, sizeof(ss_v2d) * (size_t)kSsPadSteps * 64)) != hipSuccess ||
        (e = hipMemcpy(Dv.slot, P.slot.data(), sizeof(unsigned) * P.slot.size(), hipMemcpyHostToDevice)) != hipSuccess ||
        (e = hipMemcpy(Dv.wg, P.wg.data(), sizeof(SsWg) * P.wg.size(), hipMemcpyHostToDevice)) != hipSuccess ||
        (e = hipMemcpy(Dv.win, P.win.data(), sizeof(int2) * P.win.size(), hipMemcpyHostToDevice)) != hipSuccess ||
        (e = hipMemcpy(Dv.slice_step, P.slice_step.data(), sizeof(int) * P.slice_step.size(), hipMemcpyHostToDevice)) != hipSuccess ||
        (e = hipMemcpy(Dv.slice_len, P.slice_len.data(), sizeof(int) * P.slice_len.size(), hipMemcpyHostToDevice)) != hipSuccess ||
        (ghosts && (e = hipMemcpy(Dv.wg_halo, P.wg_halo.data(), sizeof(int) * P.wg_halo.size(), hipMemcpyHostToDevice)) != hipSuccess)) {
        ss_free(Dv);
        return e;
    }
    return hipSuccess;
}

template <int D, bool NT, int ABL, int MODE>
__device__ __forceinline__ void ss_body(const SsView& S, const SsWg& W, int g, const double* __restrict__ x_in, double* __restrict__ y, const RingComm& C,
                                        double* ring , ss_v2d* s_park )
{
    constexpr bool GHOSTS = MODE == 2;
    const int tid = threadIdx.x, lane = tid & 63;
    const int wv = __builtin_amdgcn_readfirstlane(tid >> 6);
    const double* __restrict__ x = MODE != 0 ? x_in - C.n_left : x_in;
    const int r_begin = W.r_begin, r_end = W.r_end;
    if ((ABL & 8) && tid == 0) S.trace[4 * g] = __builtin_amdgcn_s_memrealtime();
    if (GHOSTS && W.link >= 0 && C.npush_runs > 0)
        for (int l = W.link; l < C.n_links; l += C.npush_runs) ring_push_link<256>(C, x_in, l);
    ss_v2d* park = s_park + wv * kSsPark * 64 + lane;
    int parked = 0, park_first = 0;
    const int t0 = wv == 0 ? W.t[0] : (wv == 1 ? W.t[1] : (wv == 2 ? W.t[2] : W.t[3]));
    const int t_end = wv == 0 ? W.t[1] : (wv == 1 ? W.t[2] : (wv == 2 ? W.t[3] : W.t[4]));
    const int clast = S.ncols - 1;
    const int cfirst = MODE != 0 ? C.n_left : 0;
    const int cowned = MODE != 0 ? C.n_left + C.n_local - 1 : clast;
    const ss_v2d* vb = S.val + lane;
    const unsigned* sb = S.slot + lane;
    ss_v2d a[D];
    unsigned sl[D];
    auto first_steps = [&]() {
#pragma unroll
        for (int d = 0; d < D; d++) {
            a[d] = NT ? __builtin_nontemporal_load(vb + (size_t)(t0 + d) * 64) : vb[(size_t)(t0 + d) * 64];
            sl[d] = sb[(size_t)(t0 + d) * 64];
        }
    };
    if (GHOSTS) {
        first_steps();
        push_wait_flags(C.flags, C.nb, C.n_nb, C.step, 0u, C.timeouts, C.spin_max, tid, 256);
        __syncthreads();
        __builtin_amdgcn_fence(__ATOMIC_ACQUIRE, "");
    }
    int r = r_begin;
    double nx[kSsNewMax / 256];
    int2 wn = make_int2(W.w1_lo, W.w1_n);
    {
        double fx[kSsFill];
#pragma unroll
        for (int u = 0; u < kSsFill; u++) fx[u] = GHOSTS ? ring_ldx<true>(x_in, C, min(W.w0_lo + tid + 256 * u, clast)) : x[min(W.w0_lo + tid + 256 * u, cowned)];
#pragma unroll
        for (int u = 0; u < kSsNewMax / 256; u++) nx[u] = (ABL & 4) ? 0.0 : x[min(max(wn.x + tid + 256 * u, cfirst), cowned)];
        if (!GHOSTS) first_steps();
// ... 119 lines not shown
```

### navierstokes_amd/mpk.py

```python
from __future__ import annotations

import ctypes
import os

import numpy as np

_HERE = os.path.dirname(os.path.abspath(__file__))
LIB_PATH = os.environ.get("MI355_SPMV_LIBRARY") or os.path.join(_HERE, "csrc", "libmi355spmv.so")

MI_OK = 0
KERNEL_AUTO, KERNEL_STREAM, KERNEL_RING, KERNEL_ROWPAR = 0, 1, 2, 3
KERNELS = {"auto": 0, "stream": 1, "ring": 2, "rowpar": 3, "bcsr4": 4, "tile": 5, "mring": 6, "sstream": 7}

_c = ctypes
_vp = ctypes.c_void_p
_LIB = None


class MiError(RuntimeError):
    def __init__(self, status, detail):
        super().__init__(f"libmi355spmv status {status}: {detail}")
        self.status = status


# ... 114 lines not shown
        "mi_bcsr4_create_layout": [i, i, _vp, _vp, _vp, i, P(_vp)],
        "mi_bcsr4_update_values_layout": [_vp, _vp, i],
        "mi_bcsr4_update_values_layout_dev": [_vp, _vp, i, _vp],
        "mi_bcsr4_spmv": [_vp, _vp, _vp],
        "mi_bcsr4_spmv_dev": [_vp, _vp, _vp, _vp],
        "mi_bcsr4_spmk": [_vp, i, _vp, _vp],
        "mi_bcsr4_spmk_dev": [_vp, i, _vp, _vp, _vp],
        "mi_bilu4_create": [i, _vp, _vp, _vp, i, i, P(_vp)],
        "mi_bilu4_create_host": [i, _vp, _vp, _vp, i, i, P(_vp)],
        "mi_bilu4_destroy": [_vp],
        "mi_bilu4_refactor": [_vp, _vp, i],
        "mi_bilu4_solve_dev": [_vp, _vp, _vp, _vp],
        "mi_bilu4_solve": [_vp, _vp, _vp],
        "mi_bilu4_info": [_vp, P(i), P(ll), P(i), P(i), P(i), P(i), P(d), P(d), P(ll)],
        "mi_bilu4_factor_host": [_vp, _vp, _vp, _vp, _vp, ll],
        "mi_bilu4_plan_probe": [i, _vp, _vp, i, P(ll), P(i), P(i), P(i), P(i), _vp, _vp, i],
        "mi_bilu4dev_plan_probe": [i, _vp, _vp, i, P(ll), P(i), P(ll)],
        "mi_bilu4dev_prepare": [_vp],
        "mi_bilu4dev_refactor": [_vp, _vp, i, _vp],
        "mi_bilu4dev_status": [_vp, P(i)],
        "mi_bilu4dev_fetch": [_vp],
        "mi_bilu4dev_info": [_vp, P(i), P(i), P(ll)],
        "mi_bilu4one_plan_probe": [i, _vp, _vp, i, i, P(i), _vp, _vp, P(ll), _vp, _vp, _vp, _vp],
        "mi_bilu4one_prepare": [_vp],
        "mi_bilu4_set_solve_form": [_vp, i],
        "mi_bilu4one_status": [_vp],
        "mi_bilu4one_info": [_vp, P(i), P(i), P(i), _vp, _vp, P(ll)],
        "mi_part_create": [i, i, _vp, _vp, _vp, _vp, P(_vp)],
        "mi_part_destroy": [_vp],
        "mi_part_sizes": [_vp, P(i), P(i), P(i), P(i)],
        "mi_part_recv_counts": [_vp, _vp],
        "mi_part_recv_ids": [_vp, i, _vp],
        "mi_part_set_send_ids": [_vp, i, i, _vp],
        "mi_part_send_counts": [_vp, _vp],
        "mi_part_local_csr": [_vp, i, P(i), P(_vp), P(_vp), P(_vp), P(_vp)],
        "mi_part_send_index": [_vp, P(i), P(_vp)],
        "mi_part_finalize": [_vp],
        "mi_part_set_kernel": [_vp, i],
        "mi_part_update_values": [_vp, _vp],
        "mi_part_pack_dev": [_vp, _vp, _vp, _vp],
        "mi_part_spmv_interior_dev": [_vp, _vp, _vp, _vp],
        "mi_part_spmv_boundary_dev": [_vp, _vp, _vp, _vp],
        "mi_comm_available": [],
        "mi_comm_unique_id": [_vp],
        "mi_part_comm_init": [_vp, _vp],
        "mi_part_comm_info": [_vp, P(i), P(i)],
        "mi_part_spmv_dev": [_vp, _vp, _vp, _vp],
        "mi_comm_selftest": [i, P(d)],
        "mi_part_send_union": [_vp, P(i), P(_vp)],
        "mi_part_allgather_setup": [_vp, _vp, _vp],
        "mi_part_set_allgather": [_vp, i],
        "mi_part_allgather_info": [_vp, P(i), P(i), P(i)],
        "mi_dist_create": [i, i, _vp, _vp, _vp, P(_vp)],
        "mi_dist_destroy": [_vp],
        "mi_dist_info": [_vp, P(i), P(i), P(i), P(i), P(ll), P(ll)],
        "mi_dist_rank_info": [_vp, i, P(i), P(ll), P(i), P(i), P(ll), P(_vp)],
        "mi_dist_update_values": [_vp, _vp],
        "mi_dist_spmv": [_vp, _vp, _vp],
        "mi_dist_spmk": [_vp, i, _vp, _vp],
        "mi_dist_dot": [_vp, _vp, _vp, P(d)],
        "mi_dist_orthogonalize": [_vp, _vp, _vp, _vp, d, P(d)],
        "mi_dist_vec_create": [_vp, P(_vp)],
        "mi_dist_vec_destroy": [_vp],
        "mi_dist_vec_set": [_vp, _vp],
        "mi_dist_vec_get": [_vp, _vp],
        "mi_dist_vec_ptr": [_vp, i, P(_vp)],
        "mi_dist_spmv_dev": [_vp, _vp, _vp],
        "mi_dist_spmk_dev": [_vp, i, _vp, _vp],
        "mi_dist_synchronize": [_vp],
        "mi_dist_dot_dev": [_vp, _vp, _vp, P(d)],
        "mi_dist_orthogonalize_dev": [_vp, _vp, _vp, _vp, d, P(d)],
    }
    for name, argt in sigs.items():
        fn = getattr(L, name)
        fn.argtypes = argt
        fn.restype = _c.c_int
    for name in ("mi_dist_exchange_name", "mi_dist_exchange_note"):
        getattr(L, name).argtypes = [_vp]
        getattr(L, name).restype = _c.c_char_p
    L.mi_part_kernel_name.argtypes = [_vp, i]
    L.mi_part_kernel_name.restype = _c.c_char_p
    for name, argt in {"mi_debug_xcc_map": [i, _vp], "mi_debug_touch_pages": [_vp, i, _vp, ll, _vp, ll],
                       "mi_part_push_debug_preset": [_vp, _c.c_uint], "mi_debug_part_push_trace": [_vp, _vp, _vp, i, _vp, P(i), _vp],
                       "mi_debug_part_ext_mode": [_vp, i], "mi_debug_part_ext_trace": [_vp, _vp, _vp, i, _vp, P(i), _vp]}.items():
        if hasattr(L, name):
            fn = getattr(L, name)
            fn.argtypes = argt
            fn.restype = _c.c_int
    _LIB = L
    return L


def check(status):
    if status != MI_OK:
        raise MiError(status, lib().mi_last_error().decode(errors="replace"))



def _is_torch(t):
    return type(t).__module__.startswith("torch")


def _stream_ptr():
    import torch

    return _vp(torch.cuda.current_stream().cuda_stream)


def _dev_ptr(t, n=None, what="vector"):
    import torch

    if not (t.is_cuda and t.dtype == torch.float64 and t.is_contiguous()):
        raise TypeError(f"{what}: expected a contiguous float64 CUDA tensor, got {t.dtype} on {t.device}")
    if n is not None and t.numel() < n:
        raise ValueError(f"{what}: needs {n} entries, has {t.numel()}")
    return _vp(t.data_ptr())


def _host_f64(a, n=None, what="vector", writable=False):
    if not isinstance(a, np.ndarray) or a.dtype != np.float64 or not a.flags.c_contiguous:
        if writable:
            raise TypeError(f"{what}: output must be a C-contiguous float64 numpy array")
        a = np.ascontiguousarray(a, dtype=np.float64)
    if n is not None and a.size < n:
        raise ValueError(f"{what}: needs {n} entries, has {a.size}")
    return a



class csrmatrix:

    def __init__(self, n, ptrow, indcol, coef, ncols=None, rowmap=None):
        self.n = int(n)
        self.ptrow = np.ascontiguousarray(ptrow, dtype=np.int32)
        self.indcol = np.ascontiguousarray(indcol, dtype=np.int32)
        self.coef = np.ascontiguousarray(coef, dtype=np.float64)
        if len(self.ptrow) != self.n + 1:
            raise ValueError("ptrow must have n+1 entries")
        self.nnz = int(self.ptrow[-1]) if self.n > 0 else 0
        self.ncols = self.n if ncols is None else int(ncols)
        self.rowmap = None if rowmap is None else np.ascontiguousarray(rowmap, dtype=np.int32)
        self._h = None
        self._kernel = KERNEL_AUTO

    @property
    def handle(self):
        if self._h is None:
            h = _vp()
            if self.rowmap is None:
                check(lib().mi_csr_create(self.n, self.ncols, self.ptrow.ctypes.data, self.indcol.ctypes.data,
                                          self.coef.ctypes.data, _c.byref(h)))
            else:
                check(lib().mi_csr_create_mapped(self.n, self.ncols, self.ptrow.ctypes.data, self.indcol.ctypes.data,
                                                 self.coef.ctypes.data, self.rowmap.ctypes.data, _c.byref(h)))
            self._h = h
            if self._kernel != KERNEL_AUTO:
                check(lib().mi_csr_set_kernel(h, self._kernel))
        return self._h

    def set_kernel(self, kernel):
        kid = KERNELS[kernel] if isinstance(kernel, str) else int(kernel)
        self._kernel = kid
        if self._h is not None:
            check(lib().mi_csr_set_kernel(self._h, kid))
        return self

    def kernel_name(self):
# ... 51 lines not shown
            buf = _PlacedBuffer(int(ptrs[k]), max(self.n, self.ncols))
            t = torch.as_tensor(buf, device="cuda")[: self.n]
            t._placed = buf
            out.append(t)
        return out, [round(us[k], 2) for k in range(nus.value)]

    def mring_info(self):
        b, r, bad, nt = _c.c_int(), _c.c_int(), _c.c_int(), _c.c_int()
        f = _c.c_double()
        us = (_c.c_double * 2)()
        check(lib().mi_csr_mring_info(self.handle, _c.byref(b), _c.byref(r), _c.byref(bad), _c.byref(f), us, _c.byref(nt)))
        return dict(built=bool(b.value), runs=r.value, runs_not_served=bad.value, nnz_fraction=f.value, us=us[0], us_nt=us[1],
                    nt=bool(nt.value))

    def sstream_info(self):
        b, r, fm = _c.c_int(), _c.c_int(), _c.c_int()
        st = _c.c_longlong()
        pad = _c.c_double()
        us = (_c.c_double * 4)()
        check(lib().mi_csr_sstream_info(self.handle, _c.byref(b), _c.byref(r), _c.byref(st), _c.byref(pad), us, _c.byref(fm)))
        return dict(built=bool(b.value), rounds=r.value, steps=st.value, padding=pad.value, us_d8_nt=us[0], us_d8_temporal=us[1], us_d12_nt=us[2],
                    us_d12_temporal=us[3], form=fm.value)

    def tile_info(self):
        b, nb, nt = _c.c_int(), _c.c_int(), _c.c_int()
        u = _c.c_double()
        us = (_c.c_double * 2)()
        check(lib().mi_csr_tile_info(self.handle, _c.byref(b), _c.byref(nb), _c.byref(u), us, _c.byref(nt)))
        return dict(built=bool(b.value), nblk=nb.value, unique_per_nnz=u.value, us=us[0], us_nt=us[1], nt=bool(nt.value))

    def reorder_info(self):
        r, b = _c.c_int(), _c.c_int()
        v = [_c.c_double() for _ in range(4)]
        check(lib().mi_csr_reorder_info(self.handle, _c.byref(r), _c.byref(b), *[_c.byref(t) for t in v]))
        return dict(reordered=bool(r.value), block=b.value, spread_before=v[0].value, spread_after=v[1].value,
                    us_natural=v[2].value, us_reordered=v[3].value)

    def spmk_info(self, k):
        e, o = _c.c_int(), _c.c_int()
        a, b = _c.c_double(), _c.c_double()
        check(lib().mi_csr_spmk_info(self.handle, int(k), _c.byref(e), _c.byref(o), _c.byref(a), _c.byref(b)))
        return dict(eligible=bool(e.value), one_launch=bool(o.value), us_k_launches=a.value, us_one_launch=b.value)

    def dot_in_epilogue(self):
        r = _c.c_int()
        check(lib().mi_csr_dot_epilogue_info(self.handle, _c.byref(r)))
        return bool(r.value)

    def dot_epilogue_layout(self):
        t, w, nb = _c.c_int(), _c.c_int(), _c.c_int()
        check(lib().mi_csr_dot_epilogue_layout(self.handle, _c.byref(t), _c.byref(w), _c.byref(nb), None, None, None, 0, 0))
        first = np.zeros(w.value + 1, np.int32)
        row0 = np.zeros(max(nb.value, 1), np.int32)
        rows = np.zeros(max(nb.value, 1), np.int32)
        check(lib().mi_csr_dot_epilogue_layout(self.handle, _c.byref(t), _c.byref(w), _c.byref(nb), first.ctypes.data,
                                               row0.ctypes.data, rows.ctypes.data, first.size, row0.size))
        return dict(threads=t.value, run_first_block=first, block_row0=row0[: nb.value], block_rows=rows[: nb.value])

    def perm(self):
        r = _c.c_int()
        p = np.empty(self.n, np.int32)
        check(lib().mi_csr_perm(self.handle, _c.byref(r), p.ctypes.data))
        return bool(r.value), p

    def to_internal(self, x, out=None):
        import torch
        out = torch.empty_like(x) if out is None else out
        check(lib().mi_vec_to_internal_dev(self.handle, _dev_ptr(x, self.n, "x"), _dev_ptr(out, self.n, "x_int"), _stream_ptr()))
        return out

    def from_internal(self, x_int, out=None):
        import torch
        out = torch.empty_like(x_int) if out is None else out
        check(lib().mi_vec_from_internal_dev(self.handle, _dev_ptr(x_int, self.n, "x_int"), _dev_ptr(out, self.n, "x"), _stream_ptr()))
        return out

    def update_values(self, coef):
        if _is_torch(coef):
            check(lib().mi_csr_update_values_dev(self.handle, _dev_ptr(coef, self.nnz, "coef"), _stream_ptr()))
        else:
            self.coef = _host_f64(coef, self.nnz, "coef")
            check(lib().mi_csr_update_values(self.handle, self.coef.ctypes.data))
        return self

    def drop_host_arrays(self):
        _ = self.handle
        self.indcol = self.indcol[:0]
        self.coef = self.coef[:0]

    def close(self):
        if self._h is not None:
            lib().mi_csr_destroy(self._h)
            self._h = None

    def __del__(self):
        try:
            self.close()
        except Exception:
            pass


class bcsr4x4_matrix:

    def __init__(self, nrows, ptrow, indcol, coef, nbcols=None, layout="row"):
        self.layout = {"row": 0, "col": 1}[layout]
        self.nrows = int(nrows)
        self.ptrow = np.ascontiguousarray(ptrow, dtype=np.int32)
        self.indcol = np.ascontiguousarray(indcol, dtype=np.int32)
        self.coef = np.ascontiguousarray(coef, dtype=np.float64)
        self.nblocks = len(self.indcol)
        self.nbcols = (int(self.indcol.max()) + 1 if self.nblocks else 0) if nbcols is None else int(nbcols)
        self.nbcols = max(self.nbcols, self.nrows)
        self._h = None

    @property
    def handle(self):
        if self._h is None:
            h = _vp()
            check(lib().mi_bcsr4_create_layout(self.nrows, self.nbcols, self.ptrow.ctypes.data, self.indcol.ctypes.data,
                                               self.coef.ctypes.data, self.layout, _c.byref(h)))
            self._h = h
        return self._h

    def update_values(self, coef):
        if _is_torch(coef):
            check(lib().mi_bcsr4_update_values_layout_dev(self.handle, _dev_ptr(coef, 16 * self.nblocks, "coef"), self.layout, _stream_ptr()))
        else:
            self.coef = _host_f64(coef, 16 * self.nblocks, "coef")
            check(lib().mi_bcsr4_update_values_layout(self.handle, self.coef.ctypes.data, self.layout))
        return self

    def close(self):
        if self._h is not None:
            lib().mi_bcsr4_destroy(self._h)
            self._h = None

    def __del__(self):
        try:
            self.close()
        except Exception:
            pass


class bilu4:

    def __init__(self, A, ptrow=None, indcol=None, coef=None, fill=0, layout="row", host_only=False):
        if isinstance(A, bcsr4x4_matrix):
            nbrows, ptrow, indcol, coef, lay = A.nrows, A.ptrow, A.indcol, A.coef, A.layout
        else:
            nbrows, lay = int(A), {"row": 0, "col": 1}[layout]
        self.nbrows = int(nbrows)
        self.layout = lay
        self.fill = int(fill)
        ptrow = np.ascontiguousarray(ptrow, dtype=np.int32)
        indcol = np.ascontiguousarray(indcol, dtype=np.int32)
        coef = _host_f64(coef, None, "coef")
        if len(ptrow) != self.nbrows + 1:
            raise ValueError("ptrow must have nbrows+1 entries")
        if coef.size < 16 * len(indcol):
            raise ValueError("coef: 16 values per block")
        self._nblocks_in = len(indcol)
        self._h = None
        h = _vp()
        make = lib().mi_bilu4_create_host if host_only else lib().mi_bilu4_create
        check(make(self.nbrows, ptrow.ctypes.data, indcol.ctypes.data, coef.ctypes.data, lay, self.fill, _c.byref(h)))
        self._h = h
# ... 679 lines not shown
```

Measured before the change: 1230.

## Skip CSR value write-back on device value updates; unfill lazily on demand

When values are updated from a device buffer and the active kernel reads only the sliced or blocked copy, the CSR coefficient array is no longer written. It is marked stale and rebuilt from the packed copy only if a CSR-based path later reads it. This removes an nnz-sized write from each value update, at the cost of new stale/read tracking and unfill kernels that every CSR reader must go through. The SpMV kernel itself is unchanged, so SpMV-only timing should see little effect.

```diff
diff --git a/include/mi355_devtools.h b/include/mi355_devtools.h
--- a/include/mi355_devtools.h
+++ b/include/mi355_devtools.h
@@ -8,6 +8,7 @@
 int mi_debug_touch_pages(mi_csr_t A, int stride_bytes, const void* d_extra0, long long bytes0, const void* d_extra1, long long bytes1);
 int mi_debug_mring_trace(mi_csr_t A, const double* d_x, double* d_y, int max_wgs, long long* host_out, int* wgs_out);
 int mi_debug_move_array(mi_csr_t A, int which, int how, unsigned long long* old_ptr, unsigned long long* new_ptr);
+int mi_debug_csr_values_state(mi_csr_t A, int* stale, int* read, long long* unfills);
 int mi_debug_mring_replan(mi_csr_t A, int skew_pct, int* table_len, int* longest_run);
 int mi_debug_part_push_trace(mi_part_t P, double* d_x_ext, double* d_y_local, int max_wgs, long long* host_out, int* wgs_out, int* halo_out);
 int mi_debug_part_ext_mode(mi_part_t P, int mode);
diff --git a/navierstokes_amd/csrc/capi_bcsr.hip b/navierstokes_amd/csrc/capi_bcsr.hip
--- a/navierstokes_amd/csrc/capi_bcsr.hip
+++ b/navierstokes_amd/csrc/capi_bcsr.hip
@@ -174,6 +174,15 @@
         hipLaunchKernelGGL((bcsr4_refresh_kernel<16384>), dim3((unsigned)std::min(grid, 256)), dim3(256), 0, s, nslices, A->nbrows, d_csr_ptrow, d_src, d_csr_out, A->d_ptrow, A->d_coef, sptr, sv);
     else
         hipLaunchKernelGGL((bcsr4_refresh_kernel<0>), dim3((unsigned)grid), dim3(256), 0, s, nslices, A->nbrows, d_csr_ptrow, d_src, d_csr_out, A->d_ptrow, A->d_coef, sptr, sv);
+    HIP_TRY(hipGetLastError());
+    return MI_OK;
+}
+
+int bcsr4_blocks_to_csr(const mi_bcsr4_s* A, const int* d_csr_ptrow, double* d_csr_out, hipStream_t s)
+{
+    if (!A || A->nbrows == 0 || A->nblocks == 0) return MI_OK;
+    const int nslices = (A->nbrows + kSellRows - 1) / kSellRows;
+    hipLaunchKernelGGL(bcsr4_blocks_to_csr_kernel, dim3((unsigned)std::max(1, std::min(nslices, 2048))), dim3(256), 0, s, nslices, A->nbrows, d_csr_ptrow, A->d_ptrow, A->d_coef, d_csr_out);
     HIP_TRY(hipGetLastError());
     return MI_OK;
 }
diff --git a/navierstokes_amd/csrc/capi_csr.hip b/navierstokes_amd/csrc/capi_csr.hip
--- a/navierstokes_amd/csrc/capi_csr.hip
+++ b/navierstokes_amd/csrc/capi_csr.hip
@@ -88,7 +88,7 @@
         T.h_wg = P.wg;
         T.fusable = P.fusable;
     }
-    sstream_fill_values(T.rounds, A->n, T.shift, A->d_ptrow, A->d_coef, nullptr, T.dev.slice_step, T.dev.slice_len, T.dev.val, T.max_slice_nnz, nullptr, T.mw ? 1 : 0);
+    sstream_fill_values(T.rounds, A->n, T.shift, A->d_ptrow, csr_values_for_read(A, nullptr), nullptr, T.dev.slice_step, T.dev.slice_len, T.dev.val, T.max_slice_nnz, nullptr, T.mw ? 1 : 0);
     if ((e = hipGetLastError()) != hipSuccess) {
         free_sstream(A);
         return fail(MI_ERR_HIP, std::string("sliced copy fill: ") + hipGetErrorString(e));
@@ -347,7 +347,7 @@
         for (void* l : losers) dfree(l);
     };
     if (blocked_choice) redraw((void**)&A->blocked->d_coef, sizeof(double) * 16 * (size_t)A->blocked->nblocks, sizeof(double) * 16, draws);
-    else redraw((void**)&A->d_coef, sizeof(double) * (size_t)nnz, sizeof(double) * (size_t)kRingPadNnz, draws);
+    else if (csr_values_for_read(A, nullptr)) redraw((void**)&A->d_coef, sizeof(double) * (size_t)nnz, sizeof(double) * (size_t)kRingPadNnz, draws);
     A->place_draws_coef = (int)A->place_us.size();
     if (A->auto_kernel == MI_KERNEL_RING) redraw((void**)&A->ring.d_slots, sizeof(unsigned short) * (size_t)A->ring.nblk * A->ring.cfg.nnzb, 0, (draws + 1) / 2);
     else if (A->auto_kernel == MI_KERNEL_MRING) redraw((void**)&A->mring.d_slots, sizeof(unsigned short) * (size_t)A->mring.nblk * kMringNnzb, 0, (draws + 1) / 2);
@@ -717,6 +717,7 @@
     if (!forced_kernel && in.nnz < kMeasureNnz && A->auto_kernel == MI_KERNEL_RING && !in.ghosts()) A->auto_kernel = MI_KERNEL_STREAM;
     if (!forced_kernel && !env_is("MI355_SPMV_AUTOTUNE", "0") && in.nnz >= kMeasureNnz && (rc = measure_at_create(A, in, defer_placement))) return rc;
     HIP_TRY(hipStreamSynchronize(nullptr));
+    A->csr_values_read = false;
     *out = owner.release();
     return MI_OK;
 }
@@ -812,7 +813,10 @@
         (hipStreamSynchronize(nullptr) != hipSuccess && (rc = fail(MI_ERR_HIP, "mi_csr_create: synchronize")))) {
         mi_csr_destroy(*out);
         *out = nullptr;
-    }
+        return rc;
+    }
+    (*out)->csr_values_read = false;
+    if ((*out)->inner) (*out)->inner->csr_values_read = false;
     return rc;
 }
 
@@ -944,6 +948,7 @@
 
 static int refresh_blocked_values(mi_csr_t A, hipStream_t s, bool sliced_done = false)
 {
+    A->csr_values_stale = false;
     if (A->ss.dev.val && !sliced_done) {
         SstreamTable& T = A->ss;
         sstream_fill_values(T.rounds, A->n, T.shift, A->d_ptrow, A->d_coef, nullptr, T.dev.slice_step, T.dev.slice_len, T.dev.val, T.max_slice_nnz, s, T.mw ? 1 : 0);
@@ -951,6 +956,22 @@
     }
     if (!A->blocked || A->blocked->nbrows == 0) return MI_OK;
     return bcsr4_refresh_from_csr(A->blocked, A->d_ptrow, A->d_coef, nullptr, s);
+}
+
+const double* csr_values_for_read(mi_csr_t A, hipStream_t s)
+{
+    A->csr_values_read = true;
+    if (A->csr_values_stale && A->d_coef) {
+        if (A->ss.dev.val) {
+            const SstreamTable& T = A->ss;
+            sstream_unfill_values(T.rounds, A->n, T.shift, A->d_ptrow, T.dev.val, T.dev.slice_step, T.dev.slice_len, A->d_coef, T.max_slice_nnz, s, T.mw ? 1 : 0);
+        } else {
+            (void)bcsr4_blocks_to_csr(A->blocked, A->d_ptrow, A->d_coef, s);
+        }
+        A->csr_unfills++;
+        if (!stream_is_capturing(s)) A->csr_values_stale = false;
+    }
+    return A->d_coef;
 }
 
 __global__ __launch_bounds__(256) void permute_values_kernel(int n, const int* __restrict__ new_ptrow, const int* __restrict__ src_start,
@@ -990,14 +1011,23 @@
         HIP_TRY(hipGetLastError());
         return refresh_blocked_values(I, s);
     }
+    const int kid = resolve_kernel(A);
+    const bool blocked_copy = A->blocked && A->blocked->nbrows > 0;
+    const bool lean = d_coef != A->d_coef && !A->csr_values_read && !stream_is_capturing(s) &&
+                      ((kid == MI_KERNEL_SSTREAM && A->ss.dev.val) || (kid == MI_KERNEL_BCSR4 && blocked_copy));
+    double* const csr_out = lean ? nullptr : A->d_coef;
     if (A->ss.dev.val && d_coef != A->d_coef) {
         SstreamTable& T = A->ss;
-        sstream_fill_values(T.rounds, A->n, T.shift, A->d_ptrow, d_coef, A->d_coef, T.dev.slice_step, T.dev.slice_len, T.dev.val, T.max_slice_nnz, s, T.mw ? 1 : 0);
+        sstream_fill_values(T.rounds, A->n, T.shift, A->d_ptrow, d_coef, csr_out, T.dev.slice_step, T.dev.slice_len, T.dev.val, T.max_slice_nnz, s, T.mw ? 1 : 0);
         HIP_TRY(hipGetLastError());
-        return refresh_blocked_values(A, s, true);
-    }
-    if (A->blocked && A->blocked->nbrows > 0 && d_coef != A->d_coef)
-        return bcsr4_refresh_from_csr(A->blocked, A->d_ptrow, d_coef, A->d_coef, s);
+        if (!lean) return refresh_blocked_values(A, s, true);
+        A->csr_values_stale = true;
+        return blocked_copy ? bcsr4_refresh_from_csr(A->blocked, A->d_ptrow, d_coef, nullptr, s) : MI_OK;
+    }
+    if (blocked_copy && d_coef != A->d_coef) {
+        A->csr_values_stale = lean;
+        return bcsr4_refresh_from_csr(A->blocked, A->d_ptrow, d_coef, csr_out, s);
+    }
     if (d_coef != A->d_coef) HIP_TRY(hipMemcpyAsync(A->d_coef, d_coef, sizeof(double) * (size_t)A->nnz, hipMemcpyDeviceToDevice, s));
     return refresh_blocked_values(A, s);
 }
diff --git a/navierstokes_amd/csrc/capi_internal.hpp b/navierstokes_amd/csrc/capi_internal.hpp
--- a/navierstokes_amd/csrc/capi_internal.hpp
+++ b/navierstokes_amd/csrc/capi_internal.hpp
@@ -200,6 +200,9 @@
     int* d_ptrow = nullptr;
     int* d_indcol = nullptr;
     double* d_coef = nullptr;
+    bool csr_values_stale = false;
+    bool csr_values_read = false;
+    long long csr_unfills = 0;
     int* d_rowmap = nullptr;
     bool mapped = false;
     int y_offset = 0;
@@ -369,6 +372,7 @@
 int csr_create_impl(int n, int ncols, const int* ptrow, const int* indcol, const double* coef, const int* rowmap, mi_csr_t* out,
                     int ghost_lo = 0, int ghost_hi = 0, bool defer_placement = false);
 int resolve_kernel(const mi_csr_s* A);
+const double* csr_values_for_read(mi_csr_t A, hipStream_t s);
 int get_table(mi_csr_t A, int nnzb, BlockTable** out);
 int launch_spmv(mi_csr_t A, const double* d_x, double* d_y, hipStream_t s, bool use_map = true, const RingComm* comm = nullptr,
                 const RingDot* dot = nullptr);
@@ -396,4 +400,5 @@
 int bcsr4_values_changed(mi_bcsr4_s* A, hipStream_t s);
 void bcsr4_drop_sliced(mi_bcsr4_s* A);
 int bcsr4_refresh_from_csr(mi_bcsr4_s* A, const int* d_csr_ptrow, const double* d_src, double* d_csr_out, hipStream_t s);
+int bcsr4_blocks_to_csr(const mi_bcsr4_s* A, const int* d_csr_ptrow, double* d_csr_out, hipStream_t s);
 int launch_bcsr4(mi_bcsr4_t A, const double* d_x, double* d_y, mi_stream_t s, bool use_map);
diff --git a/navierstokes_amd/csrc/capi_part.hip b/navierstokes_amd/csrc/capi_part.hip
--- a/navierstokes_amd/csrc/capi_part.hip
+++ b/navierstokes_amd/csrc/capi_part.hip
@@ -865,7 +865,7 @@
         BlockTable* T = nullptr;
         int rc = get_table(A, 1024, &T);
         if (rc) return rc;
-        CsrView V{A->n, A->ncols, A->d_ptrow, A->d_indcol, A->d_coef, nullptr, T->d_blk, nullptr, T->nblk};
+        CsrView V{A->n, A->ncols, A->d_ptrow, A->d_indcol, csr_values_for_read(A, s), nullptr, T->d_blk, nullptr, T->nblk};
         if (trace) hipLaunchKernelGGL((spmv_csr_fused_ext<1024, false, true>), grid, dim3(kWG), 0, s, V, d_x_ext, d_y_local, C, P->d_ext_order);
         else if (A->stream_nt) hipLaunchKernelGGL((spmv_csr_fused_ext<1024, true>), grid, dim3(kWG), 0, s, V, d_x_ext, d_y_local, C, P->d_ext_order);
         else hipLaunchKernelGGL((spmv_csr_fused_ext<1024, false>), grid, dim3(kWG), 0, s, V, d_x_ext, d_y_local, C, P->d_ext_order);
diff --git a/navierstokes_amd/csrc/devtools.hip b/navierstokes_amd/csrc/devtools.hip
--- a/navierstokes_amd/csrc/devtools.hip
+++ b/navierstokes_amd/csrc/devtools.hip
@@ -41,7 +41,7 @@
         hipLaunchKernelGGL(touch_pages_kernel, dim3(256), dim3(256), 0, nullptr, (const char*)p, bytes - 3, (size_t)stride_bytes, sink);
     };
     const size_t nnz = (size_t)A->nnz, n = (size_t)A->n;
-    touch(A->d_coef, 8 * nnz);
+    touch(csr_values_for_read(A, nullptr), 8 * nnz);
     touch(A->d_indcol, 4 * nnz);
     touch(A->d_ptrow, 4 * (n + 1));
     touch(A->d_rowmap, 4 * n);
@@ -87,7 +87,7 @@
     V.ncols = A->ncols;
     V.ptrow = A->d_ptrow;
     V.indcol = A->d_indcol;
-    V.coef = A->d_coef;
+    V.coef = csr_values_for_read(A, nullptr);
     V.rowmap = nullptr;
     V.nblk = M.nblk;
     long long* d = nullptr;
@@ -103,13 +103,23 @@
     return MI_OK;
 }
 
+extern "C" int mi_debug_csr_values_state(mi_csr_t A, int* stale, int* read, long long* unfills)
+{
+    CHECK_ARG(A, "null handle");
+    if (A->inner) A = A->inner;
+    if (stale) *stale = A->csr_values_stale ? 1 : 0;
+    if (read) *read = A->csr_values_read ? 1 : 0;
+    if (unfills) *unfills = A->csr_unfills;
+    return MI_OK;
+}
+
 extern "C" int mi_debug_move_array(mi_csr_t A, int which, int how, unsigned long long* old_ptr, unsigned long long* new_ptr)
 {
     CHECK_ARG(A && which >= 0 && which <= 3 && (how == 0 || how == 2 || how == 3), "bad argument (how = 1, hipDeviceMallocContiguous, is refused: see the comment in devtools.hip)");
     if (A->inner) A = A->inner;
     void** slot = nullptr;
     size_t bytes = 0, pad_bytes = 0;
-    if (which == 0) { slot = (void**)&A->d_coef; bytes = sizeof(double) * (size_t)A->nnz; pad_bytes = sizeof(double) * (size_t)kRingPadNnz; }
+    if (which == 0) { (void)csr_values_for_read(A, nullptr);  slot = (void**)&A->d_coef; bytes = sizeof(double) * (size_t)A->nnz; pad_bytes = sizeof(double) * (size_t)kRingPadNnz; }
     if (which == 1) { slot = (void**)&A->ring.d_slots; bytes = sizeof(unsigned short) * (size_t)A->ring.nblk * A->ring.cfg.nnzb; }
     if (which == 2) { slot = (void**)&A->d_ptrow; bytes = sizeof(int) * ((size_t)A->n + 1); pad_bytes = sizeof(int) * (size_t)kRingPadRows; }
     if (which == 3) { slot = (void**)&A->ring.d_plan; bytes = sizeof(int) * 8 * (size_t)A->ring.nblk; }
diff --git a/navierstokes_amd/csrc/launch_csr.hip b/navierstokes_amd/csrc/launch_csr.hip
--- a/navierstokes_amd/csrc/launch_csr.hip
+++ b/navierstokes_amd/csrc/launch_csr.hip
@@ -62,12 +62,12 @@
     V.ncols = A->ncols;
     V.ptrow = A->d_ptrow;
     V.indcol = A->d_indcol;
-    V.coef = A->d_coef;
     V.rowmap = use_map ? A->d_rowmap : nullptr;
     V.blk = nullptr;
     V.blk_span = nullptr;
     V.nblk = 0;
     if (kid == MI_KERNEL_BCSR4 && (((uintptr_t)d_x) & 15) == 0) return launch_bcsr4(A->blocked, d_x, d_y, (mi_stream_t)s, use_map);
+    V.coef = csr_values_for_read(A, s);
     if (kid == MI_KERNEL_BCSR4) {
         BlockTable* T = nullptr;
         int rc = get_table(A, 1024, &T);
diff --git a/navierstokes_amd/csrc/launch_spmk.hip b/navierstokes_amd/csrc/launch_spmk.hip
--- a/navierstokes_amd/csrc/launch_spmk.hip
+++ b/navierstokes_amd/csrc/launch_spmk.hip
@@ -34,14 +34,14 @@
     H->kstep_setup = 0;
 }
 
-static CsrView unmapped_view(const mi_csr_s* H)
+static CsrView unmapped_view(const mi_csr_s* H, const double* coef)
 {
     CsrView V{};
     V.n = H->n;
     V.ncols = H->ncols;
     V.ptrow = H->d_ptrow;
     V.indcol = H->d_indcol;
-    V.coef = H->d_coef;
+    V.coef = coef;
     V.rowmap = nullptr;
     V.blk = nullptr;
     V.blk_span = nullptr;
@@ -63,7 +63,7 @@
     if (maxdep > 64) return -1;
     int per_cu = 0, dev = 0, cus = 0;
     SpmkArgs dummy{};
-    if (launch_fused(H, unmapped_view(H), dummy, nullptr, true, &per_cu) != hipSuccess || hipGetDevice(&dev) != hipSuccess ||
+    if (launch_fused(H, unmapped_view(H, H->d_coef), dummy, nullptr, true, &per_cu) != hipSuccess || hipGetDevice(&dev) != hipSuccess ||
         hipDeviceGetAttribute(&cus, hipDeviceAttributeMultiprocessorCount, dev) != hipSuccess) {
         (void)hipGetLastError();
         return -1;
@@ -121,7 +121,7 @@
     static const unsigned spin_max = 1u << (getenv("MI355_SPMK_SPIN_LOG2") ? std::max(8, std::min(30, atoi(getenv("MI355_SPMK_SPIN_LOG2")))) : 21);
     K.spin_max = spin_max;
     K.acquire = env_is("MI355_SPMK_ACQUIRE", "1") ? 1 : 0;
-    hipError_t e = launch_fused(H, unmapped_view(H), K, s);
+    hipError_t e = launch_fused(H, unmapped_view(H, csr_values_for_read(H, s)), K, s);
     if (e != hipSuccess) return fail(MI_ERR_HIP, std::string("one-launch powers step: ") + hipGetErrorString(e));
     return MI_OK;
 }
diff --git a/navierstokes_amd/csrc/spmv_bcsr_sell.hpp b/navierstokes_amd/csrc/spmv_bcsr_sell.hpp
--- a/navierstokes_amd/csrc/spmv_bcsr_sell.hpp
+++ b/navierstokes_amd/csrc/spmv_bcsr_sell.hpp
@@ -150,6 +150,27 @@
                     v.y = at(4 * r + q, 4 * j + 2 * h + 1);
                 }
                 reinterpret_cast<sell_v2d*>(sell_val + (size_t)(t0 + j) * kSellStepDoubles)[h * 64 + lane] = v;
+            }
+        }
+        __syncthreads();
+    }
+}
+
+__global__ __launch_bounds__(256) void bcsr4_blocks_to_csr_kernel(int nslices, int nbrows, const int* __restrict__ csr_ptrow, const int* __restrict__ bptr,
+                                                                  const double* __restrict__ bval, double* __restrict__ csr_out)
+{
+    __shared__ int rp[4 * kSellRows + 1];
+    __shared__ int bp[kSellRows + 1];
+    const int tid = threadIdx.x;
+    for (int s = blockIdx.x; s < nslices; s += gridDim.x) {
+        if (tid <= 4 * kSellRows) rp[tid] = csr_ptrow[min(4 * kSellRows * s + tid, 4 * nbrows)];
+        if (tid <= kSellRows) bp[tid] = bptr[min(kSellRows * s + tid, nbrows)];
+        __syncthreads();
+        for (int r = 0; r < kSellRows; r++) {
+            const int nb = bp[r + 1] - bp[r];
+            for (int k = tid; k < 16 * nb; k += 256) {
+                const int q = k / (4 * nb), pos = k - 4 * nb * q;
+                csr_out[rp[4 * r + q] + pos] = bval[16 * (size_t)(bp[r] + (pos >> 2)) + 4 * q + (pos & 3)];
             }
         }
         __syncthreads();
diff --git a/navierstokes_amd/csrc/spmv_sstream.hpp b/navierstokes_amd/csrc/spmv_sstream.hpp
--- a/navierstokes_amd/csrc/spmv_sstream.hpp
+++ b/navierstokes_amd/csrc/spmv_sstream.hpp
@@ -353,6 +353,57 @@
         hipLaunchKernelGGL((sstream_fill_kernel<0>), dim3((unsigned)std::min(nslices, 2048)), dim3(256), 0, s, nslices, n, shift, d_ptrow, d_src, d_csr_out, d_slice_step, d_slice_len, d_val, pair64);
 }
 
+template <int CAP>
+__global__ __launch_bounds__(256) void sstream_unfill_kernel(int nslices, int n, int shift, const int* __restrict__ ptrow, const ss_v2d* __restrict__ val,
+                                                             const int* __restrict__ slice_step, const int* __restrict__ slice_len,
+                                                             double* __restrict__ csr_out, int pair64)
+{
+    __shared__ double buf[CAP > 0 ? CAP : 1];
+    __shared__ int rp[kSsSliceRows + 1];
+    const int tid = threadIdx.x;
+    for (int sidx = blockIdx.x; sidx < nslices; sidx += gridDim.x) {
+        const int row0 = kSsSliceRows * sidx - shift;
+        if (tid <= kSsSliceRows) rp[tid] = ptrow[max(0, min(row0 + tid, n))];
+        __syncthreads();
+        const int base = rp[0], seg = rp[kSsSliceRows] - base;
+        const bool staged = CAP > 0 && seg <= CAP;
+        const int t0 = slice_step[sidx], L = slice_len[sidx];
+        for (int q = tid; q < L * 64; q += 256) {
+            const int j = q >> 6, lane = q & 63;
+            const int ra = pair64 ? lane : 2 * lane, rb = pair64 ? lane + 64 : 2 * lane + 1;
+            const int a0 = rp[ra], na = rp[ra + 1] - a0, b0 = rp[rb], nb = rp[rb + 1] - b0;
+            if (j >= na && j >= nb) continue;
+            const ss_v2d v = val[(size_t)(t0 + j) * 64 + lane];
+            if (j < na) {
+                if (staged) buf[a0 - base + j] = v.x;
+                else csr_out[a0 + j] = v.x;
+            }
+            if (j < nb) {
+                if (staged) buf[b0 - base + j] = v.y;
+                else csr_out[b0 + j] = v.y;
+            }
+        }
+        if (staged) {
+            __syncthreads();
+            for (int k = tid; k < seg; k += 256) csr_out[base + k] = buf[k];
+        }
+        __syncthreads();
+    }
+}
+
+inline void sstream_unfill_values(int rounds, int n, int shift, const int* d_ptrow, const ss_v2d* d_val, const int* d_slice_step, const int* d_slice_len,
+                                  double* d_csr_out, int max_slice_nnz, hipStream_t s, int pair64 = 0)
+{
+    const int nslices = 4 * rounds;
+    if (nslices <= 0) return;
+    if (max_slice_nnz <= 2048)
+        hipLaunchKernelGGL((sstream_unfill_kernel<2048>), dim3((unsigned)std::min(nslices, 2048)), dim3(256), 0, s, nslices, n, shift, d_ptrow, d_val, d_slice_step, d_slice_len, d_csr_out, pair64);
+    else if (max_slice_nnz <= 8192)
+        hipLaunchKernelGGL((sstream_unfill_kernel<8192>), dim3((unsigned)std::min(nslices, 1024)), dim3(256), 0, s, nslices, n, shift, d_ptrow, d_val, d_slice_step, d_slice_len, d_csr_out, pair64);
+    else
+        hipLaunchKernelGGL((sstream_unfill_kernel<0>), dim3((unsigned)std::min(nslices, 2048)), dim3(256), 0, s, nslices, n, shift, d_ptrow, d_val, d_slice_step, d_slice_len, d_csr_out, pair64);
+}
+
 struct SsDevice {
     ss_v2d* val = nullptr;
     unsigned* slot = nullptr;
diff --git a/navierstokes_amd/mpk.py b/navierstokes_amd/mpk.py
--- a/navierstokes_amd/mpk.py
+++ b/navierstokes_amd/mpk.py
@@ -220,7 +220,9 @@
     L.mi_part_kernel_name.restype = _c.c_char_p
     for name, argt in {"mi_debug_xcc_map": [i, _vp], "mi_debug_touch_pages": [_vp, i, _vp, ll, _vp, ll],
                        "mi_part_push_debug_preset": [_vp, _c.c_uint], "mi_debug_part_push_trace": [_vp, _vp, _vp, i, _vp, P(i), _vp],
-                       "mi_debug_part_ext_mode": [_vp, i], "mi_debug_part_ext_trace": [_vp, _vp, _vp, i, _vp, P(i), _vp]}.items():
+                       "mi_debug_part_ext_mode": [_vp, i], "mi_debug_part_ext_trace": [_vp, _vp, _vp, i, _vp, P(i), _vp],
+                       "mi_debug_csr_values_state": [_vp, P(i), P(i), P(ll)],
+                       "mi_debug_move_array": [_vp, i, i, P(_c.c_ulonglong), P(_c.c_ulonglong)]}.items():
         if hasattr(L, name):
             fn = getattr(L, name)
             fn.argtypes = argt
@@ -438,6 +440,15 @@
             self.coef = _host_f64(coef, self.nnz, "coef")
             check(lib().mi_csr_update_values(self.handle, self.coef.ctypes.data))
         return self
+
+    def values_state(self):
+        L = lib()
+        if not hasattr(L, "mi_debug_csr_values_state"):
+            raise RuntimeError("mi_debug_csr_values_state lives in libmi355spmv_dev.so only (MI355_SPMV_LIBRARY)")
+        st, rd = _c.c_int(), _c.c_int()
+        un = _c.c_longlong()
+        check(L.mi_debug_csr_values_state(self.handle, _c.byref(st), _c.byref(rd), _c.byref(un)))
+        return dict(stale=st.value, read=rd.value, unfills=un.value)
 
     def drop_host_arrays(self):
         _ = self.handle
```

New measurement: 1230 (median of 2 runs). About the same (-0.0%).
